# 294coder/Dif-PAN

Measured on AMD Instinct MI355X. Metric: fused megapixels/sec at T=1000, WV3 64x64x8 tiles, higher is better.
Workload: dtype f32-class (f16x2 split); 1 GPU; WV3 pansharpening, batch 64 of 64x64x8 tiles per GPU, T=1000 DDPM p_sample, fp32; tiles_per_gpu=64, tiles_total=64, T=1000, model_evaluations=1000, sampler=ddpm, parallelism=tile-shard x1, launches_per_denoising_step=132

## Files before the change

### dif-pan_amd/csrc/ddif_la.cpp

```cpp
#include "ddif_plan.h"
#include "kernels_lafuse.h"
#include "kernels_lafuse8.h"

namespace ddif {

namespace {
template <int TH, int TW, int NBQ, int NBA>
int la_launch1(const LaFuseArgs& a, int grid, hipStream_t s, bool prepare_only) {
    using G = LaFuseGeom<TH, TW, NBQ, NBA>;
    auto fn = linattn_fused_kernel<TH, TW, NBQ, NBA>;
    if (prepare_only) {
        DDIF_HIPCHK(hipFuncSetAttribute(reinterpret_cast<const void*>(fn), hipFuncAttributeMaxDynamicSharedMemorySize, (int)G::smem));
        return 0;
    }
    hipLaunchKernelGGL(fn, dim3(grid), dim3(2 * TH * TW), G::smem, s, a);
    return 0;
}
template <int TH, int TW>
int la_launch_t(const LaFuseArgs& a, int nbq, int nba, int grid, hipStream_t s, bool prep) {
    switch (nbq * 10 + nba) {
        case 21: return la_launch1<TH, TW, 2, 1>(a, grid, s, prep);
        case 31: return la_launch1<TH, TW, 3, 1>(a, grid, s, prep);
        case 41: return la_launch1<TH, TW, 4, 1>(a, grid, s, prep);
        case 22: return la_launch1<TH, TW, 2, 2>(a, grid, s, prep);
        case 32: return la_launch1<TH, TW, 3, 2>(a, grid, s, prep);
        case 42: return la_launch1<TH, TW, 4, 2>(a, grid, s, prep);
        case 62:
            if constexpr (TH == 16) return la_launch1<TH, TW, 6, 2>(a, grid, s, prep);
            [[fallthrough]];
        default: return fail(DDIF_ERR_INVALID, "linattn_fused: no instantiation for %d q blocks / %d output blocks", nbq, nba);
    }
}
}

bool lafuse_supported(int H, int fea, int dout) {
    static const bool la6 = env_flag("DDIF_LA6", true);
    if (H == 16 && fea == 192 && dout == 64 && la6) return true;
    return (H == 64 || H == 32 || H == 16) && fea % 32 == 0 && fea >= 64 && fea <= 128 && dout % 32 == 0 && dout >= 32 && dout <= 64;
}
int lafuse_strip(int H, int nw) { return 32 * nw / H; }
int lafuse_launch(const LaFuseArgs& a, int grid, hipStream_t s, bool prepare_only, int nw) {
    const int nbq = (a.c0 + a.c1) / 32, nba = a.dout / 32;
    if (nw == 4) {
        if (a.H == 64) return la_launch_t<64, 2>(a, nbq, nba, grid, s, prepare_only);
        if (a.H == 32) return la_launch_t<32, 4>(a, nbq, nba, grid, s, prepare_only);
        if (a.H == 16) return la_launch_t<16, 8>(a, nbq, nba, grid, s, prepare_only);
    } else {
        if (a.H == 64) return la_launch_t<64, 4>(a, nbq, nba, grid, s, prepare_only);
        if (a.H == 32) return la_launch_t<32, 8>(a, nbq, nba, grid, s, prepare_only);
        if (a.H == 16) return la_launch_t<16, 16>(a, nbq, nba, grid, s, prepare_only);
    }
    return fail(DDIF_ERR_INVALID, "linattn_fused: H = %d", a.H);
}

bool lafuse8_supported(int H, int W, int c0, int c1, int dout) {
    return H == 8 && W == 8 && c0 % 64 == 0 && c1 % 64 == 0 && (c0 + c1 == 256 || c0 + c1 == 192) && dout == 128;
}
int lafuse8_launch(const LaFuseArgs& a, int grid, hipStream_t s, bool prepare_only) {
    const int nbq = (a.c0 + a.c1) / 32;
    if (nbq == 8) {
        auto fn = linattn8_fused_kernel<8>;
        if (prepare_only) {
            DDIF_HIPCHK(hipFuncSetAttribute(reinterpret_cast<const void*>(fn), hipFuncAttributeMaxDynamicSharedMemorySize, (int)LaFuse8Geom<8>::smem));
            return 0;
        }
        hipLaunchKernelGGL(fn, dim3(grid), dim3(512), LaFuse8Geom<8>::smem, s, a);
        return 0;
    }
    if (nbq == 6) {
        auto fn = linattn8_fused_kernel<6>;
        if (prepare_only) {
            DDIF_HIPCHK(hipFuncSetAttribute(reinterpret_cast<const void*>(fn), hipFuncAttributeMaxDynamicSharedMemorySize, (int)LaFuse8Geom<6>::smem));
            return 0;
        }
        hipLaunchKernelGGL(fn, dim3(grid), dim3(512), LaFuse8Geom<6>::smem, s, a);
        return 0;
    }
    return fail(DDIF_ERR_INVALID, "linattn8_fused: %d feature channels", a.c0 + a.c1);
}

}
```

### dif-pan_amd/csrc/ddif_net.cpp

```cpp
#include "ddif_net.h"
#include <cstdint>
#include <tuple>
#include "kernels_refresh.h"

namespace ddif {

thread_local std::string g_err;

int fail(int code, const char* fmt, ...) {
    char buf[1024];
    va_list ap;
    va_start(ap, fmt);
    vsnprintf(buf, sizeof(buf), fmt, ap);
    va_end(ap);
    g_err = buf;
    return code;
}

static bool in_list(const int32_t* a, int n, int v) {
    for (int i = 0; i < n; ++i)
        if (a[i] == v) return true;
    return false;
}

// ... 96 lines not shown
    size_t n = 1;
    for (int i = 0; i < ndim; ++i) {
        if (shape[i] < 0) return fail(DDIF_ERR_INVALID, "ddif_net_load(%s): negative dim", key);
        t.shape.push_back(shape[i]);
        n *= (size_t)shape[i];
    }
    t.v.assign(data, data + n);
    host[key] = std::move(t);
    committed = false;
    return 0;
}

int64_t Net::num_params() const {
    int64_t n = 0;
    for (auto& kv : host)
        if (kv.first != "noise_level_mlp.0.freqs") n += (int64_t)kv.second.v.size();
    return n;
}

namespace {

struct Blob {
    std::vector<float> v;
    size_t add(const float* p, size_t n) {
        size_t off = (v.size() + 63) & ~(size_t)63;
        v.resize(off + n, 0.f);
        if (p) std::memcpy(v.data() + off, p, n * sizeof(float));
        return off;
    }
};

size_t pack_conv(Blob& b, const float* w, int cout, int cin, int ks, int ck, int* n_chunks_out) {
    const int n_chunks = (cin + ck - 1) / ck, nb = (cout + 31) / 32, nb_pad = (nb + 3) & ~3;
    const int taps = ks * ks, K8 = ck / 8;
    const size_t n = (size_t)nb_pad * n_chunks * taps * K8 * 256;
    const size_t off = b.add(nullptr, n);
    float* o = b.v.data() + off;
    for (int nbi = 0; nbi < nb; ++nbi)
        for (int ch = 0; ch < n_chunks; ++ch)
            for (int tap = 0; tap < taps; ++tap)
                for (int k8 = 0; k8 < K8; ++k8)
                    for (int h = 0; h < 2; ++h)
                        for (int j = 0; j < 32; ++j)
                            for (int i = 0; i < 4; ++i) {
                                const int ci = ch * ck + k8 * 8 + 4 * h + i, co = nbi * 32 + j;
                                float val = 0.f;
                                if (co < cout && ci < cin) val = w[((size_t)co * cin + ci) * taps + tap];
                                o[(((((size_t)nbi * n_chunks + ch) * taps + tap) * K8 + k8) * 2 + h) * 128 + j * 4 + i] = val;
                            }
    *n_chunks_out = n_chunks;
    return off;
}

inline unsigned bf16_bits_host(float x) {
    unsigned u;
    std::memcpy(&u, &x, 4);
    return (u + 0x7fffu + ((u >> 16) & 1u)) >> 16;
}
inline float bf16_val_host(unsigned b) {
    const unsigned u = b << 16;
    float f;
    std::memcpy(&f, &u, 4);
    return f;
}
size_t pack_conv_x3(Blob& b, const float* w, int cout, int cin, int ks, int ck) {
    const int taps = ks * ks, K16 = ck / 16;
    const int n_chunks = (cin + ck - 1) / ck, nb = (cout + 31) / 32, nb_pad = (nb + 3) & ~3;
    const size_t per = (size_t)taps * K16 * 3 * 256;
    const size_t off = b.add(nullptr, (size_t)nb_pad * n_chunks * per);
    uint16_t* o = reinterpret_cast<uint16_t*>(b.v.data() + off);
    for (int nbi = 0; nbi < nb; ++nbi)
        for (int ch = 0; ch < n_chunks; ++ch)
            for (int tap = 0; tap < taps; ++tap)
              for (int k16 = 0; k16 < K16; ++k16)
                for (int h = 0; h < 2; ++h)
                    for (int j = 0; j < 32; ++j)
                        for (int t = 0; t < 8; ++t) {
                            const int ci = ch * ck + 16 * k16 + 8 * h + t, co = nbi * 32 + j;
                            float val = 0.f;
                            if (co < cout && ci < cin) val = w[((size_t)co * cin + ci) * taps + tap];
                            unsigned q[3];
                            q[0] = bf16_bits_host(val);
                            const float r1 = val - bf16_val_host(q[0]);
                            q[1] = bf16_bits_host(r1);
                            q[2] = bf16_bits_host(r1 - bf16_val_host(q[1]));
                            for (int pl = 0; pl < 3; ++pl) {
                                const size_t fl = (((((size_t)nbi * n_chunks + ch) * taps + tap) * K16 + k16) * 3 + pl) * 256 + (size_t)(h * 32 + j) * 4;
                                o[fl * 2 + t] = (uint16_t)q[pl];
                            }
                        }
    return off;
}

inline uint16_t f16_bits_host(float x) {
    const _Float16 hv = (_Float16)x;
    uint16_t b;
    std::memcpy(&b, &hv, 2);
    return b;
}
inline float f16_val_host(uint16_t b) {
    _Float16 hv;
    std::memcpy(&hv, &b, 2);
    return (float)hv;
}
size_t pack_conv_f16(Blob& b, const float* w, int cout, int cin, int ks, int ck) {
    const int taps = ks * ks, K16 = ck / 16;
    for (size_t i = 0; i < (size_t)cout * cin * taps; ++i)
        if (!(std::fabs(w[i]) <= DDIF_F16_WMAX)) return (size_t)-1;
    const int n_chunks = (cin + ck - 1) / ck, nb = (cout + 31) / 32, nb_pad = (nb + 3) & ~3;
    const size_t per = (size_t)taps * K16 * 2 * 256;
    const size_t off = b.add(nullptr, (size_t)nb_pad * n_chunks * per);
    uint16_t* o = reinterpret_cast<uint16_t*>(b.v.data() + off);
    for (int nbi = 0; nbi < nb; ++nbi)
        for (int ch = 0; ch < n_chunks; ++ch)
            for (int tap = 0; tap < taps; ++tap)
                for (int k16 = 0; k16 < K16; ++k16)
                    for (int h = 0; h < 2; ++h)
                        for (int j = 0; j < 32; ++j)
                            for (int t = 0; t < 8; ++t) {
                                const int ci = ch * ck + 16 * k16 + 8 * h + t, co = nbi * 32 + j;
                                float val = 0.f;
                                if (co < cout && ci < cin) val = w[((size_t)co * cin + ci) * taps + tap] * DDIF_F16_WSCALE;
                                uint16_t q[2];
                                q[0] = f16_bits_host(val);
                                q[1] = f16_bits_host(val - f16_val_host(q[0]));
                                for (int pl = 0; pl < 2; ++pl) {
                                    const size_t fl = (((((size_t)nbi * n_chunks + ch) * taps + tap) * K16 + k16) * 2 + pl) * 256 + (size_t)(h * 32 + j) * 4;
                                    o[fl * 2 + t] = q[pl];
                                }
                            }
    return off;
}

size_t pack_conv_b1(Blob& b, size_t x3_off, int cout, int cin, int ks, int ck) {
    const size_t steps = (size_t)((((cout + 31) / 32 + 3) & ~3)) * ((cin + ck - 1) / ck) * (ks * ks) * (ck / 16);
    const size_t off = b.add(nullptr, steps * 256);
    for (size_t st = 0; st < steps; ++st) std::memcpy(b.v.data() + off + st * 256, b.v.data() + x3_off + st * 3 * 256, 256 * sizeof(float));
    return off;
}

}

int Net::commit(hipStream_t stream) {
    Blob b;
    struct PendConv { std::string name; size_t w_off; long bias_off; int cin, cout, ks, ck, n_chunks; long x3_off = -1; long f16_off = -1; long b1_off = -1; };
    std::vector<PendConv> pend;
    std::map<std::string, size_t> vec_off;
    std::string missing;
    recipes.clear();
    auto rec_pack = [&](int kind, const std::string& s0, const std::string& s1, size_t off, int cout, int cin0, int cin1, int ks, int ck, int n_chunks) {
        Recipe r;
        r.kind = kind;
        r.src0 = s0;
        r.src1 = s1;
        r.dst_off = off;
        r.cout = cout;
        r.cin0 = cin0;
        r.cin1 = cin1;
        r.ks = ks;
        r.ck = ck;
        r.n_chunks = n_chunks;
        const size_t nb_pad = (size_t)(((cout + 31) / 32 + 3) & ~3);
        r.n_out = kind == RF_PACK_F32 ? nb_pad * n_chunks * ks * ks * (ck / 8) * 256 : nb_pad * n_chunks * ks * ks * (ck / 16) * 3 * 256;
        recipes.push_back(r);
    };
    auto rec_copy = [&](int kind, const std::string& s0, const std::string& s1, size_t off, size_t n, int C = 0) {
        Recipe r;
        r.kind = kind;
        r.src0 = s0;
        r.src1 = s1;
        r.dst_off = off;
        r.n_out = n;
        r.cout = C;
        recipes.push_back(r);
    };

    auto need = [&](const std::string& key) -> const HostTensor* {
        const HostTensor* t = get(key);
        if (!t && missing.empty()) missing = key;
        return t;
    };
    auto add_conv = [&](const std::string& name, bool has_bias) {
        const HostTensor* w = need(name + ".weight");
        const HostTensor* bs = has_bias ? need(name + ".bias") : nullptr;
        if (!w || (has_bias && !bs)) return;
        if (w->shape.size() != 4) { if (missing.empty()) missing = name + ".weight (expected 4-d)"; return; }
        PendConv p;
        p.name = name;
        p.cout = (int)w->shape[0];
        p.cin = (int)w->shape[1];
        p.ks = (int)w->shape[2];
        p.ck = (p.ks == 3 || p.cin <= 16) ? 16 : 32;
        p.w_off = pack_conv(b, w->v.data(), p.cout, p.cin, p.ks, p.ck, &p.n_chunks);
        rec_pack(RF_PACK_F32, name + ".weight", "", p.w_off, p.cout, p.cin, 0, p.ks, p.ck, p.n_chunks);
        if (p.ck % 16 == 0 && (p.ks == 3 || p.ck == 32)) {
            p.x3_off = (long)pack_conv_x3(b, w->v.data(), p.cout, p.cin, p.ks, p.ck);
            rec_pack(RF_PACK_X3, name + ".weight", "", (size_t)p.x3_off, p.cout, p.cin, 0, p.ks, p.ck, p.n_chunks);
            p.f16_off = (long)pack_conv_f16(b, w->v.data(), p.cout, p.cin, p.ks, p.ck);
            p.b1_off = (long)pack_conv_b1(b, (size_t)p.x3_off, p.cout, p.cin, p.ks, p.ck);
        }
        p.bias_off = bs ? (long)b.add(bs->v.data(), bs->v.size()) : -1;
        if (bs) rec_copy(RF_COPY, name + ".bias", "", (size_t)p.bias_off, bs->v.size());
        pend.push_back(p);
    };
    auto add_vec = [&](const std::string& key) {
        const HostTensor* t = need(key);
        if (t) {
            vec_off[key] = b.add(t->v.data(), t->v.size());
            rec_copy(RF_COPY, key, "", vec_off[key], t->v.size());
        }
    };
    auto add_dw = [&](const std::string& key) {
        const HostTensor* t = need(key);
        if (!t) return;
        const int C = (int)t->shape[0];
        std::vector<float> r((size_t)9 * C);
        for (int c = 0; c < C; ++c)
            for (int k = 0; k < 9; ++k) r[(size_t)k * C + c] = t->v[(size_t)c * 9 + k];
        vec_off[key] = b.add(r.data(), r.size());
        rec_copy(RF_DW, key, "", vec_off[key], r.size(), C);
    };
    auto add_resblock = [&](const std::string& p) {
        add_vec(p + ".block1.block.0.weight");
        add_vec(p + ".block1.block.0.bias");
        add_conv(p + ".block1.block.3", true);
        add_vec(p + ".block2.block.0.weight");
        add_vec(p + ".block2.block.0.bias");
        add_conv(p + ".block2.block.3", true);
    };
    auto add_attn = [&](const std::string& p) {
        add_vec(p + ".norm.weight");
        add_vec(p + ".norm.bias");
        add_conv(p + ".qkv", false);
        add_conv(p + ".out", true);
    };

    std::vector<float> wall_h, ball_h;
    std::vector<std::tuple<std::string, size_t, size_t, size_t, size_t>> slot_keys;
    slot_off.clear();
    nslots = 0;
    auto add_slot = [&](const std::string& rb) {
        const HostTensor* w = need(rb + ".noise_func.noise_func.0.weight");
        const HostTensor* bs = need(rb + ".noise_func.noise_func.0.bias");
        if (!w || !bs) return;
        slot_off[rb] = nslots;
        slot_keys.emplace_back(rb, wall_h.size(), (size_t)nslots, w->v.size(), bs->v.size());
        wall_h.insert(wall_h.end(), w->v.begin(), w->v.end());
        ball_h.insert(ball_h.end(), bs->v.begin(), bs->v.end());
        nslots += (int)bs->v.size();
    };

    for (auto& L : downs) {
        if (L.kind == L_STEM) add_conv(L.p, true);
        else if (L.kind == L_DOWN) add_conv(L.p + ".conv", true);
        else {
            add_slot(L.p + ".res_block");
            add_resblock(L.p + ".res_block");
            if (L.attn) add_attn(L.p + ".attn");
            add_conv(L.p + ".cond_inj.body.0", false);
            add_vec(L.p + ".cond_inj.body.1.weight");
            add_vec(L.p + ".cond_inj.body.1.bias");
            add_conv(L.p + ".cond_inj.body.3", true);
            add_conv(L.p + ".cond_inj.x_conv", true);
            if (const HostTensor* wx = get(L.p + ".cond_inj.x_conv.weight")) {
                if (wx->shape.size() == 4 && wx->shape[1] == 32 && wx->shape[0] % 32 == 0 && wx->shape[2] == 1) {
                    const int co = (int)wx->shape[0];
                    std::vector<float> r((size_t)co * 32);
                    for (int nb = 0; nb < co / 32; ++nb)
                        for (int ln = 0; ln < 64; ++ln)
                            for (int sx = 0; sx < 16; ++sx)
                                r[((size_t)nb * 64 + ln) * 16 + sx] = wx->v[(size_t)(32 * nb + (ln & 31)) * 32 + 8 * (sx >> 2) + 4 * (ln >> 5) + (sx & 3)];
                    vec_off[L.p + ".cond_inj.x_conv.xf"] = b.add(r.data(), r.size());
                }
            }
        }
    }
    for (auto& L : mid) {
        add_slot(L.p + ".res_block");
        add_resblock(L.p + ".res_block");
        if (L.attn) add_attn(L.p + ".attn");
    }
    for (auto& L : ups) {
        if (L.kind == L_UP) { add_conv(L.p + ".conv", true); continue; }
        add_slot(L.p + ".res_block");
        add_resblock(L.p + ".res_block");
        if (L.attn) add_attn(L.p + ".attn");
        const std::string ci = L.p + ".cond_inj";
        add_vec(ci + ".prenorm_x.weight");
        add_vec(ci + ".prenorm_x.bias");
        add_dw(ci + ".q.0.weight");
        add_conv(ci + ".q.1", true);
        add_dw(ci + ".kv.0.weight");
        add_conv(ci + ".kv.1", true);
        const HostTensor *wo = need(ci + ".attn_out.weight"), *bo = need(ci + ".attn_out.bias");
        const HostTensor* wr = get(ci + ".attn_res.weight");
        const HostTensor* br = get(ci + ".attn_res.bias");
        if (wo) {
            vec_off[ci + ".attn_out.weight"] = b.add(wo->v.data(), wo->v.size());
            rec_copy(RF_COPY, ci + ".attn_out.weight", "", vec_off[ci + ".attn_out.weight"], wo->v.size());
        }
        if (wr) {
            vec_off[ci + ".attn_res.weight"] = b.add(wr->v.data(), wr->v.size());
            rec_copy(RF_COPY, ci + ".attn_res.weight", "", vec_off[ci + ".attn_res.weight"], wr->v.size());
        }
        if (wo && bo) {
            const int co = (int)wo->shape[0], fea = (int)wo->shape[1];
            PendConv p;
            p.name = ci + ".attn_mix";
            p.cout = co;
            p.ks = 1;
            std::vector<float> bsum(bo->v);
            if (wr && br) {
                std::vector<float> cat((size_t)co * 2 * fea);
                for (int o = 0; o < co; ++o) {
                    std::memcpy(&cat[(size_t)o * 2 * fea], &wo->v[(size_t)o * fea], fea * sizeof(float));
                    std::memcpy(&cat[(size_t)o * 2 * fea + fea], &wr->v[(size_t)o * fea], fea * sizeof(float));
                    bsum[o] = bo->v[o] + br->v[o];
                }
                p.cin = 2 * fea;
                p.ck = 32;
                p.w_off = pack_conv(b, cat.data(), co, p.cin, 1, p.ck, &p.n_chunks);
                rec_pack(RF_PACK_F32, ci + ".attn_out.weight", ci + ".attn_res.weight", p.w_off, co, fea, fea, 1, p.ck, p.n_chunks);
                p.x3_off = (long)pack_conv_x3(b, cat.data(), co, p.cin, 1, p.ck);
                rec_pack(RF_PACK_X3, ci + ".attn_out.weight", ci + ".attn_res.weight", (size_t)p.x3_off, co, fea, fea, 1, p.ck, p.n_chunks);
                p.b1_off = (long)pack_conv_b1(b, (size_t)p.x3_off, co, p.cin, 1, p.ck);
            } else {
                p.cin = fea;
                p.ck = fea <= 16 ? 16 : 32;
                p.w_off = pack_conv(b, wo->v.data(), co, fea, 1, p.ck, &p.n_chunks);
                rec_pack(RF_PACK_F32, ci + ".attn_out.weight", "", p.w_off, co, fea, 0, 1, p.ck, p.n_chunks);
                if (p.ck == 32) {
                    p.x3_off = (long)pack_conv_x3(b, wo->v.data(), co, fea, 1, p.ck);
                    rec_pack(RF_PACK_X3, ci + ".attn_out.weight", "", (size_t)p.x3_off, co, fea, 0, 1, p.ck, p.n_chunks);
                    p.b1_off = (long)pack_conv_b1(b, (size_t)p.x3_off, co, fea, 1, p.ck);
                }
            }
            p.bias_off = (long)b.add(bsum.data(), bsum.size());
            if (wr && br) rec_copy(RF_SUM, ci + ".attn_out.bias", ci + ".attn_res.bias", (size_t)p.bias_off, bsum.size());
            else rec_copy(RF_COPY, ci + ".attn_out.bias", "", (size_t)p.bias_off, bsum.size());
            pend.push_back(p);
        }
        add_conv(ci + ".ffn.0", false);
        add_conv(ci + ".ffn.2", false);
        add_conv(ci + ".ffn.3", true);
        {
            const HostTensor *w2 = get(ci + ".ffn.2.weight"), *w3 = get(ci + ".ffn.3.weight"), *b3 = get(ci + ".ffn.3.bias");
            if (w2 && w3 && b3 && w2->shape.size() == 4 && w3->shape.size() == 4 && w3->shape[1] == w2->shape[0] && w3->shape[2] == 1) {
                const int co = (int)w3->shape[0], mid = (int)w2->shape[0], cin = (int)w2->shape[1];
                std::vector<float> wm((size_t)co * cin * 9);
                std::vector<double> row((size_t)cin * 9);
                for (int o = 0; o < co; ++o) {
                    std::fill(row.begin(), row.end(), 0.0);
                    for (int k = 0; k < mid; ++k) {
                        const double a = (double)w3->v[(size_t)o * mid + k];
                        const float* src = &w2->v[(size_t)k * cin * 9];
                        for (int e = 0; e < cin * 9; ++e) row[e] += a * (double)src[e];
                    }
                    for (int e = 0; e < cin * 9; ++e) wm[(size_t)o * cin * 9 + e] = (float)row[e];
                }
                PendConv p;
                p.name = ci + ".ffn.23";
                p.cout = co;
                p.cin = cin;
                p.ks = 3;
                p.ck = 16;
                p.w_off = pack_conv(b, wm.data(), co, cin, 3, p.ck, &p.n_chunks);
                p.x3_off = (long)pack_conv_x3(b, wm.data(), co, cin, 3, p.ck);
                p.f16_off = (long)pack_conv_f16(b, wm.data(), co, cin, 3, p.ck);
                p.b1_off = (long)pack_conv_b1(b, (size_t)p.x3_off, co, cin, 3, p.ck);
                p.bias_off = (long)b.add(b3->v.data(), b3->v.size());
                pend.push_back(p);
            }
        }
    }
    add_vec("final_conv.block.0.weight");
    add_vec("final_conv.block.0.bias");
    add_conv("final_conv.block.3", true);

    const HostTensor *hw1 = need("noise_level_mlp.1.weight"), *hb1 = need("noise_level_mlp.1.bias");
    const HostTensor *hw3 = need("noise_level_mlp.3.weight"), *hb3 = need("noise_level_mlp.3.bias");
    if (!missing.empty()) return fail(DDIF_ERR_MISSING, "ddif_net_commit: weight '%s' was never loaded", missing.c_str());

    const int half = cfg.inner_channel / 2;
    std::vector<float> fr(half);
    if (const HostTensor* f = get("noise_level_mlp.0.freqs")) {
        if ((int)f->v.size() != half) return fail(DDIF_ERR_INVALID, "noise_level_mlp.0.freqs must have %d entries", half);
        fr = f->v;
    } else {
        const float k = -(float)std::log(1e4);
        for (int j = 0; j < half; ++j) fr[j] = std::exp(k * ((float)j / (float)half));
    }
    const size_t o_fr = b.add(fr.data(), fr.size());
    const size_t o_w1 = b.add(hw1->v.data(), hw1->v.size()), o_b1 = b.add(hb1->v.data(), hb1->v.size());
    const size_t o_w3 = b.add(hw3->v.data(), hw3->v.size()), o_b3 = b.add(hb3->v.data(), hb3->v.size());
    const size_t o_wall = b.add(wall_h.data(), wall_h.size()), o_ball = b.add(ball_h.data(), ball_h.size());
    rec_copy(RF_COPY, "noise_level_mlp.1.weight", "", o_w1, hw1->v.size());
    rec_copy(RF_COPY, "noise_level_mlp.1.bias", "", o_b1, hb1->v.size());
    rec_copy(RF_COPY, "noise_level_mlp.3.weight", "", o_w3, hw3->v.size());
    rec_copy(RF_COPY, "noise_level_mlp.3.bias", "", o_b3, hb3->v.size());
    for (auto& sk : slot_keys) {
        rec_copy(RF_COPY, std::get<0>(sk) + ".noise_func.noise_func.0.weight", "", o_wall + std::get<1>(sk), std::get<3>(sk));
        rec_copy(RF_COPY, std::get<0>(sk) + ".noise_func.noise_func.0.bias", "", o_ball + std::get<2>(sk), std::get<4>(sk));
    }
    merged_stale = false;
    last_ptrs.clear();
    refresh_keys.clear();
    dconv.clear();
    dgrad_filled = false;
    if (blob || dgrad_blob) {
        for (hipEvent_t e : reader_events) DDIF_HIPCHK(hipEventSynchronize(e));
        DDIF_HIPCHK(hipStreamSynchronize(stream));
    }
    if (dgrad_blob) {
        DDIF_HIPCHK(hipFree(dgrad_blob));
        dgrad_blob = nullptr;
    }

    if (blob) {
        DDIF_HIPCHK(hipFree(blob));
        blob = nullptr;
    }
    blob_floats = b.v.size() + 64;
    DDIF_HIPCHK(hipMalloc((void**)&blob, blob_floats * sizeof(float)));
    DDIF_HIPCHK(hipMemcpy(blob, b.v.data(), b.v.size() * sizeof(float), hipMemcpyHostToDevice));
    (void)stream;

    conv.clear();
    vec.clear();
    for (auto& p : pend) {
        PackedConv pc;
        pc.w = blob + p.w_off;
        pc.w_x3 = p.x3_off >= 0 ? blob + p.x3_off : nullptr;
        pc.w_f16 = p.f16_off >= 0 ? blob + p.f16_off : nullptr;
        pc.w_b1 = p.b1_off >= 0 ? blob + p.b1_off : nullptr;
        pc.bias = p.bias_off >= 0 ? blob + p.bias_off : nullptr;
        pc.cin = p.cin;
        pc.cout = p.cout;
        pc.ks = p.ks;
        pc.ck = p.ck;
        pc.n_chunks = p.n_chunks;
        conv[p.name] = pc;
    }
    vec_absmax.clear();
    for (auto& kv : vec_off) {
        vec[kv.first] = blob + kv.second;
        float m = 0.f;
        if (const HostTensor* t = get(kv.first))
            for (float x : t->v) m = std::fabs(x) > m || std::isnan(x) ? (std::isnan(x) ? INFINITY : std::fabs(x)) : m;
        vec_absmax[blob + kv.second] = m;
    }
    freqs = blob + o_fr;
    w1 = blob + o_w1;
    b1 = blob + o_b1;
    w3 = blob + o_w3;
    b3 = blob + o_b3;
    wall = blob + o_wall;
    ball = blob + o_ball;
    committed = true;
    ++generation;
    return 0;
}

int Net::refresh_device(int n, const char* const* keys, const float* const* ptrs, hipStream_t stream) {
    if (!committed) return fail(DDIF_ERR_STATE, "ddif_net_refresh: ddif_net_commit has not been called");
    if (n < 1 || !keys || !ptrs) return fail(DDIF_ERR_INVALID, "ddif_net_refresh: bad arguments");
#ifndef DDIF_EMU
    for (hipEvent_t e : reader_events) (void)hipStreamWaitEvent(stream, e, 0);
#endif
    bool same = (int)refresh_keys.size() == n && d_recs != nullptr;
    for (int i = 0; i < n && same; ++i) {
        if (!keys[i] || !ptrs[i]) return fail(DDIF_ERR_INVALID, "ddif_net_refresh: NULL key / pointer at %d", i);
        same = refresh_in_ptrs[i] == ptrs[i] && refresh_keys[i] == keys[i];
    }
    if (same) {
        hipLaunchKernelGGL(refresh_blob_kernel, dim3((unsigned)refresh_blocks), dim3(256), 0, stream, (const RefreshRec*)d_recs, n_recs);
        DDIF_HIPCHK(hipGetLastError());
        merged_stale = true;
        if (dgrad_blob) dgrad_filled = true;
        return 0;
    }
    std::map<std::string, const float*> by_key;
    for (int i = 0; i < n; ++i) {
        if (!keys[i] || !ptrs[i]) return fail(DDIF_ERR_INVALID, "ddif_net_refresh: NULL key / pointer at %d", i);
        by_key[keys[i]] = ptrs[i];
    }
    refresh_keys.clear();
    std::vector<const float*> flat;
    flat.reserve(recipes.size() * 2);
    for (auto& r : recipes) {
        auto i0 = by_key.find(r.src0);
        if (i0 == by_key.end()) return fail(DDIF_ERR_MISSING, "ddif_net_refresh: parameter '%s' was not given", r.src0.c_str());
        const float* p1 = nullptr;
        if (!r.src1.empty()) {
            auto i1 = by_key.find(r.src1);
            if (i1 == by_key.end()) return fail(DDIF_ERR_MISSING, "ddif_net_refresh: parameter '%s' was not given", r.src1.c_str());
            p1 = i1->second;
        }
        flat.push_back(i0->second);
        flat.push_back(p1);
    }
    if (flat != last_ptrs || !d_recs) {
        std::vector<RefreshRec> recs(recipes.size());
        long long blk = 0;
        for (size_t k = 0; k < recipes.size(); ++k) {
            const Recipe& r = recipes[k];
            RefreshRec& d = recs[k];
            d.kind = r.kind;
            d.src0 = flat[2 * k];
            d.src1 = flat[2 * k + 1];
            d.dst = (r.dblob ? dgrad_blob : blob) + r.dst_off;
            d.tr = r.tr;
            d.fc0 = r.fc0;
            d.fc1 = r.fc1;
            d.cout = r.cout;
            d.cin0 = r.cin0;
            d.cin1 = r.cin1;
            d.ks = r.ks;
            d.ck = r.ck;
            d.n_chunks = r.n_chunks;
            d.n_out = (long long)r.n_out;
            d.blk0 = blk;
            blk += (long long)((r.n_out + 255) / 256);
        }
        if (d_recs) {
            DDIF_HIPCHK(hipStreamSynchronize(stream));
            DDIF_HIPCHK(hipFree(d_recs));
            d_recs = nullptr;
        }
        DDIF_HIPCHK(hipMalloc(&d_recs, recs.size() * sizeof(RefreshRec)));
        DDIF_HIPCHK(hipMemcpy(d_recs, recs.data(), recs.size() * sizeof(RefreshRec), hipMemcpyHostToDevice));
        n_recs = (int)recs.size();
        refresh_blocks = blk;
        last_ptrs = flat;
    }
    refresh_keys.assign(keys, keys + n);
    refresh_in_ptrs.assign(ptrs, ptrs + n);
    hipLaunchKernelGGL(refresh_blob_kernel, dim3((unsigned)refresh_blocks), dim3(256), 0, stream, (const RefreshRec*)d_recs, n_recs);
    DDIF_HIPCHK(hipGetLastError());
    merged_stale = true;
    if (dgrad_blob) dgrad_filled = true;
    return 0;
}

int Net::build_dgrad_packs() {
    if (!committed) return fail(DDIF_ERR_STATE, "build_dgrad_packs: ddif_net_commit has not been called");
    if (dgrad_blob) return 0;
    size_t off = 0;
    std::vector<Recipe> extra;
    auto add = [&](const std::string& name, const std::string& s0, const std::string& s1, int cout_f, int fc0, int fc1, int ks) {
        PackedConv pc;
        pc.cin = cout_f;
        pc.cout = (fc0 + fc1 + 3) & ~3;
        pc.ks = ks;
        pc.ck = (ks == 3 || pc.cin <= 16) ? 16 : 32;
        pc.n_chunks = (pc.cin + pc.ck - 1) / pc.ck;
        const size_t nb_pad = (size_t)(((pc.cout + 31) / 32 + 3) & ~3);
        const bool x3 = pc.ck % 16 == 0 && (ks == 3 || pc.ck == 32);
        Recipe r;
        r.kind = RF_PACK_F32;
        r.src0 = s0;
        r.src1 = s1;
        r.cout = pc.cout;
        r.cin0 = cout_f;
        r.ks = ks;
        r.ck = pc.ck;
        r.n_chunks = pc.n_chunks;
        r.tr = 1;
        r.fc0 = fc0;
        r.fc1 = fc1;
        r.dblob = true;
        r.dst_off = off;
        r.n_out = nb_pad * pc.n_chunks * ks * ks * (pc.ck / 8) * 256;
        const size_t w_off = off;
        off += (r.n_out + 63) & ~(size_t)63;
        extra.push_back(r);
        size_t x3_off = 0;
        if (x3) {
            Recipe q = r;
            q.kind = RF_PACK_X3;
            q.dst_off = off;
            q.n_out = nb_pad * pc.n_chunks * ks * ks * (pc.ck / 16) * 3 * 256;
            x3_off = off;
            off += (q.n_out + 63) & ~(size_t)63;
            extra.push_back(q);
        }
        pc.w = reinterpret_cast<const float*>(w_off + 1);
        pc.w_x3 = x3 ? reinterpret_cast<const float*>(x3_off + 1) : nullptr;
        pc.bias = nullptr;
        dconv[name] = pc;
    };
    for (auto& kv : conv) {
        const std::string& name = kv.first;
        const PackedConv& f = kv.second;
        const size_t n = name.size();
        auto ends = [&](const char* suf) { const size_t m = strlen(suf); return n >= m && name.compare(n - m, m, suf) == 0; };
        if (ends(".ffn.23") || ends(".body.0") || name == "downs.0") continue;
        if (ends(".attn_mix")) {
            const std::string ci = name.substr(0, n - strlen(".attn_mix"));
            const bool has_res = get(ci + ".attn_res.weight") != nullptr;
            const int fea = has_res ? f.cin / 2 : f.cin;
            add(name, ci + ".attn_out.weight", has_res ? ci + ".attn_res.weight" : "", f.cout, fea, has_res ? fea : 0, 1);
            continue;
        }
        add(name, name + ".weight", "", f.cout, f.cin, 0, f.ks);
    }
    dgrad_floats = off + 64;
// ... 16 lines not shown
```

### dif-pan_amd/csrc/ddif_plan.cpp

```cpp
#include "ddif_plan.h"
#include <algorithm>
#include "kernels_conv.h"
#include "kernels_misc.h"
#include "attn_args.h"
#include "quantile_args.h"
#include "kernels_lafuse.h"

namespace ddif {

ConvVariant get_conv_variant(int ks, int stride, int ups, int ck, int pro, int cfg, int vec, int epi, int math) {
    if (cfg == 20 || cfg == 21)
        return (stride == 1 && !ups && vec == 1) ? get_lr_variant(ks, cfg == 20 ? 2 : 4, pro, epi, (math == MATH_F16X2 && pro == PRO_COLSM) ? MATH_BF16X3 : math) : ConvVariant();
    if (ks == 1) return get_conv_variant_k1(stride, ups, ck, pro, cfg, vec, epi);
    if (ks == 3) return epi ? get_conv_variant_k3e(stride, ups, ck, pro, cfg, vec, epi) : get_conv_variant_k3(stride, ups, ck, pro, cfg, vec);
    return ConvVariant();
}

static int num_cus();
static int x3_enabled() { static const int v = env_int("DDIF_X3", 1); return v; }
static int f16_enabled() { static const int v = env_int("DDIF_F16", 1); return v; }
int g_math_mode = [] { const char* e = getenv("DDIF_MATH"); return (e && std::strcmp(e, "bf16") == 0) ? 1 : 0; }();
int g_f16_raw = env_flag("DDIF_F16_RAW", true);
static int lr_rows_enabled() { static const int v = env_int("DDIF_LR_ROWS", 1); return v; }
static int lafuse_enabled() { static const int v = env_int("DDIF_LAFUSE", 1); return v; }
// ... 917 lines not shown
        s.stats = true;
        s.name = "up";
        const Tensor uin = cur;
        DDIF_TRY(p.add_conv(step, s, &cur));
        --lev;
        if (train) tmod(Plan::TrainMod::UP, L.p + ".conv", uin, cur);
        return 0;
    }
    struct Dec {
        std::string ci;
        Tensor skip;
        int skip_from = -1;
        int fea = 0, d = 0, Hl = 0, Wl = 0, cd = 0;
        size_t pre_dec0 = 0;
        float* ctx = nullptr;
        Tensor kdw, kv;
        const float *pn_g = nullptr, *pn_b = nullptr, *q0w = nullptr;
    };
    int decoder_context(Dec& D) {
        const int BB = B, fea = D.fea, d = D.d, Hl = D.Hl, Wl = D.Wl, cd = D.cd;
        D.pre_dec0 = pre.size();
        DDIF_TRY(p.alloc_tensor(&D.kdw, cd, Hl, Wl));
        {
            DwArgs a{};
            a.in0 = p.cdec[lev].p;
            a.c0 = cd;
            a.B = B;
            a.H = Hl;
            a.W = Wl;
            a.w = V(D.ci + ".kv.0.weight");
            if (!a.w) return fail(DDIF_ERR_MISSING, "%s.kv.0.weight missing", D.ci.c_str());
            a.out_dw = D.kdw.p;
            a.tiles_x = (Wl + 15) / 16;
            a.tiles_y = (Hl + 7) / 8;
            Op op;
            op.name = "kv.dw3x3";
            op.flop = 2.0 * 9 * B * Hl * Wl * cd;
            op.bytes = 8.0 * B * Hl * Wl * cd;
            op.run = [a](hipStream_t s, const StepCtx&) { launch_dw3x3(s, a); };
            pre.push_back(std::move(op));
        }
        ConvSpec s;
        DDIF_TRY(need_conv(D.ci + ".kv.1", &s.pc));
        s.in0 = D.kdw;
        s.name = "kv.1x1";
        DDIF_TRY(p.add_conv(pre, s, &D.kv));
        if (train) return 0;
        float *kmx = nullptr, *ksm = nullptr, *ctx = nullptr;
        DDIF_TRY(p.dalloc(&kmx, (size_t)B * Hl * fea));
        DDIF_TRY(p.dalloc(&ksm, (size_t)B * Hl * fea));
        DDIF_TRY(p.dalloc(&ctx, (size_t)B * 8 * d * d));
        D.ctx = ctx;
        const Tensor kv = D.kv;
        {
            Op op;
            op.name = "k.softmax_stats";
            op.bytes = 8.0 * B * Hl * Wl * fea;
            op.run = [kv, kmx, ksm, fea, BB, Hl, Wl](hipStream_t s, const StepCtx&) {
                hipLaunchKernelGGL(softmax_stats_kernel, ew_grid((size_t)BB * Hl * fea), dim3(256), 0, s, (const float*)kv.p, 2 * fea, 0, fea, BB, Hl, Wl, 1, kmx, ksm);
            };
            pre.push_back(std::move(op));
        }
        {
            Op op;
            op.name = "linattn_ctx";
            op.flop = 2.0 * B * 8 * d * d * (double)Hl * Wl;
            op.bytes = 4.0 * B * Hl * Wl * 2.0 * fea;
            op.run = [kv, kmx, ksm, ctx, fea, d, BB, Hl, Wl](hipStream_t s, const StepCtx&) {
                hipLaunchKernelGGL(linattn_ctx_kernel, dim3(8, BB), dim3(256), 2 * 32 * d * sizeof(float), s, (const float*)kv.p, (const float*)kmx, (const float*)ksm, BB, Hl, Wl, fea, d, ctx);
            };
            pre.push_back(std::move(op));
        }
        return 0;
    }
    DwArgs gn_dw_args(const Dec& D, Tensor dwq, Tensor xn) const {
        DwArgs a{};
        a.in0 = cur.p;
        a.c0 = cur.C;
        a.in1 = D.skip.p;
        a.c1 = D.skip.C;
        a.B = B;
        a.H = D.Hl;
        a.W = D.Wl;
        a.st0 = cur.st;
        a.np0 = cur.np;
        a.st1 = D.skip.st;
        a.np1 = D.skip.np;
        a.gamma = D.pn_g;
        a.beta = D.pn_b;
        a.w = D.q0w;
        a.out_dw = dwq.p;
        a.out_xn = xn.p;
        a.use_gn = 1;
        return a;
    }
    void pack_mix_weights(const Dec& D, const float* wo, const float* wr, float* wmix, int co_n, int ck, int nch, int nb_pad, size_t per, bool x3) {
        Op op;
        op.name = "pack_mix_weights";
        const float scale = 1.0f / std::sqrt((float)D.d);
        const int BB = B, fea = D.fea, d = D.d;
        const float* ctx = D.ctx;
        op.flop = 2.0 * B * co_n * (double)fea * d;
        op.run = [wo, wr, ctx, wmix, BB, co_n, fea, d, scale, ck, nch, nb_pad, per, x3](hipStream_t s, const StepCtx&) {
            if (x3) hipLaunchKernelGGL(pack_mix_weights_x3_kernel, ew_grid(per * BB), dim3(256), 0, s, wo, wr, (const float*)ctx, BB, co_n, fea, d, scale, ck, nch, nb_pad, wmix);
            else hipLaunchKernelGGL(pack_mix_weights_kernel, ew_grid(per * BB), dim3(256), 0, s, wo, wr, (const float*)ctx, BB, co_n, fea, d, scale, ck, nch, nb_pad, wmix);
        };
        pre.push_back(std::move(op));
    }
    int ffn_train(const Dec& D, Tensor a, Tensor* f0, Tensor* f1, Tensor* f2, Tensor* f3c) {
        const int Hl = D.Hl, Wl = D.Wl;
        ConvSpec s;
        DDIF_TRY(need_conv(D.ci + ".ffn.0", &s.pc));
        s.in0 = a;
        s.use_bias = false;
        s.name = "ffn.0 (train)";
        DDIF_TRY(p.add_conv(step, s, f0));
        DDIF_TRY(p.alloc_tensor(f1, f0->C, f0->H, f0->W, true));
        Op op;
        op.name = "silu";
        op.cls = cls_small(Hl * Wl, 5);
        op.bytes = 8.0 * B * Hl * Wl * f0->C;
        Tensor ff0 = *f0, ff1 = *f1;
        const size_t n = (size_t)B * Hl * Wl * f0->C;
        op.run = [ff0, ff1, n](hipStream_t st, const StepCtx&) { tk::silu_fwd(st, ff0.p, n, ff1.p); };
        step.push_back(std::move(op));
        ConvSpec s2;
        DDIF_TRY(need_conv(D.ci + ".ffn.2", &s2.pc));
        s2.in0 = *f1;
        s2.use_bias = false;
        s2.name = "ffn.2 (train)";
        DDIF_TRY(p.add_conv(step, s2, f2));
        ConvSpec s3;
        DDIF_TRY(need_conv(D.ci + ".ffn.3", &s3.pc));
        s3.in0 = *f2;
        s3.name = "ffn.3 (train)";
        return p.add_conv(step, s3, f3c);
    }
    int droppath_add(Tensor f3c, Tensor a, Tensor* out, float** scale_out) {
        Tensor f3;
        float* scale = nullptr;
        DDIF_TRY(p.alloc_tensor(&f3, f3c.C, f3c.H, f3c.W, true));
        DDIF_TRY(p.dalloc(&scale, (size_t)B));
        p.path_sites.push_back(scale);
        const int HW = f3c.H * f3c.W, Cc = f3c.C, BB = B;
        int chunks = (HW * Cc / 4 + 256 * 8 - 1) / (256 * 8);
        if (chunks < 1) chunks = 1;
        f3.np = chunks;
        DDIF_TRY(p.dalloc(&f3.st, (size_t)B * chunks * 2));
        Op op;
        op.name = "droppath_add";
        op.cls = cls_small(HW, 5);
        op.bytes = 12.0 * B * HW * Cc;
        op.run = [f3c, scale, a, f3, HW, Cc, BB, chunks](hipStream_t s, const StepCtx&) {
            hipLaunchKernelGGL(droppath_add_kernel, dim3(chunks, BB), dim3(256), 64, s, (const float*)f3c.p, (const float*)scale, (const float*)a.p, HW, Cc, f3.p, f3.st);
        };
        step.push_back(std::move(op));
        *out = f3;
        *scale_out = scale;
        return 0;
    }
    int decoder_block_train(const Dec& D, Tensor* out) {
        const std::string& ci = D.ci;
        const int BB = B, fea = D.fea, d = D.d, Hl = D.Hl, Wl = D.Wl;
        const PackedConv* pq1t = PC(ci + ".q.1");
        const PackedConv* pmixt = PC(ci + ".attn_mix");
        if (!pq1t || !pmixt) return fail(DDIF_ERR_MISSING, "%s: q.1 / attn_out missing", ci.c_str());
        if (!cur.st || !D.skip.st) return fail(DDIF_ERR_STATE, "%s: prenorm without producer statistics", ci.c_str());
        if (!D.pn_g || !D.pn_b || !D.q0w) return fail(DDIF_ERR_MISSING, "%s: prenorm/q.0 weights missing", ci.c_str());
        Tensor xn, dwq, q, o, a, f0, f1, f2, f3c, f3, kdw_pad;
        float *la_ctx = nullptr, *la_part = nullptr;
        DDIF_TRY(p.alloc_tensor(&xn, fea, Hl, Wl, true));
        DDIF_TRY(p.alloc_tensor(&dwq, fea, Hl, Wl, true));
        {
            DwArgs da = gn_dw_args(D, dwq, xn);
            da.tiles_x = (Wl + 15) / 16;
            da.tiles_y = (Hl + 7) / 8;
            Op op;
            op.name = "q.gn_dw3x3 (train)";
            op.cls = cls_small(Hl * Wl, 5);
            op.flop = 2.0 * 9 * B * Hl * Wl * fea;
            op.bytes = 12.0 * B * Hl * Wl * fea;
            op.run = [da](hipStream_t s, const StepCtx&) { launch_dw3x3(s, da); };
            step.push_back(std::move(op));
        }
        {
            ConvSpec s;
            s.pc = pq1t;
            s.in0 = dwq;
            s.name = "q.1x1 (train)";
            DDIF_TRY(p.add_conv(step, s, &q));
        }
        DDIF_TRY(p.alloc_tensor(&o, fea, Hl, Wl, true));
        {
            Op op;
            op.name = "linattn_fwd";
            op.cls = cls_small(Hl * Wl, 5);
            op.flop = 4.0 * B * 8 * d * d * (double)Hl * Wl;
            op.bytes = 16.0 * B * Hl * Wl * fea;
            Tensor qq = q, kk = D.kv, oo = o;
            if ((Hl > Wl ? Hl : Wl) * fea > 8192 || d > 32 || d % 4)
                return fail(DDIF_ERR_INVALID, "%s: train-mode linear attention holds one image line x %d channels in LDS: lines of more than %d pixels are not supported",
                            ci.c_str(), fea, 8192 / fea);
            DDIF_TRY(p.dalloc(&la_ctx, (size_t)B * fea * d));
            DDIF_TRY(p.dalloc(&la_part, tk::linattn_part_floats(B, Hl, Wl, fea, d)));
            float *cx = la_ctx, *pt = la_part;
            {
                Op pc;
                pc.name = "linattn_ctx (train)";
                pc.bytes = 8.0 * B * Hl * Wl * fea;
                pc.run = [kk, BB, d, Hl, Wl, cx, pt](hipStream_t s, const StepCtx&) { tk::linattn_ctx(s, kk.p, BB, 8, d, Hl, Wl, cx, pt); };
                pre.push_back(std::move(pc));
                for (size_t i = D.pre_dec0; i < pre.size(); ++i) pre[i].side = true;
            }
            op.run = [qq, oo, BB, d, Hl, Wl, fea, cx](hipStream_t s, const StepCtx&) { tk::linattn_apply(s, qq.p, cx, BB, 8, d, Hl, Wl, oo.p, fea); };
            step.push_back(std::move(op));
        }
        const bool has_res = pmixt->cin == 2 * fea;
        {
            ConvSpec s;
            s.pc = pmixt;
            s.in0 = o;
            if (has_res) s.in1 = xn;
            else s.res = xn.p;
            s.name = "attn_out+res (train)";
            DDIF_TRY(p.add_conv(step, s, &a));
        }
        DDIF_TRY(ffn_train(D, a, &f0, &f1, &f2, &f3c));
        float* scale = nullptr;
        DDIF_TRY(droppath_add(f3c, a, &f3, &scale));
        DDIF_TRY(p.alloc_tensor(&kdw_pad, (D.cd + 3) & ~3, Hl, Wl));
        Plan::TrainMod& m = tmod(Plan::TrainMod::DEC, ci, cur, f3);
        m.t[0] = D.skip;
        m.t[1] = xn;
        m.t[2] = dwq;
        m.t[3] = q;
        m.t[4] = D.kv;
        m.t[5] = D.kdw;
        m.t[6] = kdw_pad;
        m.t[7] = o;
        m.t[8] = a;
        m.t[9] = f0;
        m.t[10] = f1;
        m.t[11] = f2;
        m.scale = scale;
        m.ctx = la_ctx;
        m.la_part = la_part;
        m.has_res = has_res;
        m.skip_from = D.skip_from;
        m.lev = lev;
        *out = f3;
        return 0;
    }
    int linattn_fused(const Dec& D, const PackedConv* pq1, Tensor* amix, bool* fused) {
        const std::string& ci = D.ci;
        const int fea = D.fea, Hl = D.Hl, Wl = D.Wl;
        const Tensor& skip = D.skip;
        *fused = false;
        const PackedConv* pm = PC(ci + ".attn_mix");
        const float* wr = V(ci + ".attn_res.weight");
        const bool la8 = la8_enabled() && lafuse8_supported(Hl, Wl, cur.C, skip.C, pm ? pm->cout : 0);
        bool ok = lafuse_enabled() && f16_enabled() && x3_enabled() && lr_enabled() && pm && wr && pq1->w_f16 && pq1->bias && pm->bias && (Hl * Wl >= 256 || la8) &&
                  pq1->cout == fea && pq1->ck == 32 && pm->ck == 32 && pm->cin == 2 * fea && cur.C % 16 == 0 && skip.C % 16 == 0 && (la8 || lafuse_supported(Hl, fea, pm->cout));
        if (ok) {
            auto ig = net.vec_absmax.find(D.pn_g), ib = net.vec_absmax.find(D.pn_b), iw = net.vec_absmax.find(D.q0w);
            ok = ig != net.vec_absmax.end() && ib != net.vec_absmax.end() && iw != net.vec_absmax.end() &&
                 (std::sqrt((double)fea * Hl * Wl) * ig->second + ib->second) * 9.0 * iw->second < DDIF_F16_AMAX;
        }
        if (!ok) return 0;
        const float* wo = V(ci + ".attn_out.weight");
        if (!wo) return fail(DDIF_ERR_MISSING, "%s.attn_out.weight missing", ci.c_str());
        const int nb_pad = (((pm->cout + 31) / 32) + 3) & ~3;
        const size_t per = (size_t)nb_pad * pm->n_chunks * 2 * 3 * 256;
        float* wmix = nullptr;
        DDIF_TRY(p.dalloc(&wmix, per * B));
        pack_mix_weights(D, wo, wr, wmix, pm->cout, 32, pm->n_chunks, nb_pad, per, true);
        p.use(cur.p);
        p.use(skip.p);
        DDIF_TRY(p.alloc_tensor(amix, pm->cout, Hl, Wl, true));
        LaFuseArgs a{};
        a.xcd = (xcd_mask() & 4) ? 1 : 0;
        a.in0 = cur.p;
        a.c0 = cur.C;
        a.in1 = skip.p;
        a.c1 = skip.C;
        a.B = B;
        a.H = Hl;
        a.W = Wl;
        a.st0 = cur.st;
        a.np0 = cur.np;
        a.st1 = skip.st;
        a.np1 = skip.np;
        a.gamma = D.pn_g;
        a.beta = D.pn_b;
        a.dw_w = D.q0w;
        a.wq = pq1->w_f16;
        a.nchq = pq1->n_chunks;
        a.bq = pq1->bias;
        a.wmix = wmix;
        a.wmix_bstride = (long long)per;
        a.nch_mix = pm->n_chunks;
        a.bias = pm->bias;
        a.out = amix->p;
        a.dout = pm->cout;
        int la_nw = 8;
        if (!la8) {
            static const int nw_env = env_int("DDIF_LA_NW", 0);
            const long wg8 = (long)B * ((Wl + lafuse_strip(Hl, 8) - 1) / lafuse_strip(Hl, 8));
            la_nw = nw_env == 4 || nw_env == 8 ? nw_env : (wg8 < num_cus() ? 4 : 8);
        }
        if (!p.dry) DDIF_TRY(la8 ? lafuse8_launch(a, 1, nullptr, true) : lafuse_launch(a, 1, nullptr, true, la_nw));
        const int nstrips = la8 ? 2 : (Wl + lafuse_strip(Hl, la_nw) - 1) / lafuse_strip(Hl, la_nw);
        long cap = num_cus();
        if (g_debug_grid_cap > 0 && g_debug_grid_cap < cap) cap = g_debug_grid_cap;
        Op op;
        op.name = la8 ? "linattn8_fused" : "linattn_fused";
        {
            char lb[160];
            snprintf(lb, sizeof lb, "linattn_fused GN+dw3x3+q.1+softmax_H+attn_out+res %d+%d->%d @%dx%d", cur.C, skip.C, pm->cout, Hl, Wl);
            op.label = lb;
        }
        op.flop = 2.0 * B * Hl * Wl * ((double)fea * fea + 9.0 * fea + 2.0 * fea * pm->cout);
        op.bytes = 4.0 * B * Hl * Wl * ((double)fea + pm->cout);
        op.cls = cls_small(Hl * Wl, 1);
        op.mfma_w = (3.0 * fea * fea + 6.0 * 2.0 * fea * pm->cout) / ((double)fea * fea + 9.0 * fea + 2.0 * fea * pm->cout);
        op.run = [a, nstrips, cap, la8, la_nw](hipStream_t st, const StepCtx&) {
            const long nw = (long)a.B * nstrips;
            if (la8) (void)lafuse8_launch(a, (int)(nw < cap ? nw : cap), st, false);
            else (void)lafuse_launch(a, (int)(nw < cap ? nw : cap), st, false, la_nw);
        };
        step.push_back(std::move(op));
        *fused = true;
        return 0;
    }
    int q_low_resolution(const Dec& D, const PackedConv* pq1, Tensor xn, Tensor* q, float** qmx, float** qsm) {
        const int BB = B, fea = D.fea, Hl = D.Hl, Wl = D.Wl;
        Tensor dwq;
        DDIF_TRY(p.alloc_tensor(&dwq, fea, Hl, Wl, true));
        p.use(cur.p);
        p.use(D.skip.p);
        p.use(xn.p);
        DwArgs a = gn_dw_args(D, dwq, xn);
        Op op;
        op.name = "q.gn_dw3x3";
        op.cls = 2;
        {
            char lb[160];
            snprintf(lb, sizeof lb, "q.gn_dw3x3 %d+%d @%dx%d", cur.C, D.skip.C, Hl, Wl);
            op.label = lb;
        }
        op.flop = 2.0 * 9 * B * Hl * Wl * fea;
        op.bytes = 4.0 * B * Hl * Wl * 3.0 * fea;
        const size_t sm = (size_t)(Hl + 2) * (Wl + 2) * 36 * sizeof(float);
        if (sm > 64 * 1024) DDIF_HIPCHK(hipFuncSetAttribute(reinterpret_cast<const void*>(gn_dw3x3_small_kernel), hipFuncAttributeMaxDynamicSharedMemorySize, (int)sm));
        a.xcd = (xcd_mask() & 8) ? 1 : 0;
        const dim3 gdw = a.xcd ? dim3(BB, (fea + 31) / 32) : dim3((fea + 31) / 32, BB);
        op.run = [a, gdw, sm](hipStream_t s, const StepCtx&) { hipLaunchKernelGGL(gn_dw3x3_small_kernel, gdw, dim3(256), sm, s, a); };
        step.push_back(std::move(op));
        ConvSpec s;
        s.pc = pq1;
        s.in0 = dwq;
        s.name = "q.1x1";
        if (Hl <= 16) {
            DDIF_TRY(p.dalloc(qmx, (size_t)B * Wl * fea));
            DDIF_TRY(p.dalloc(qsm, (size_t)B * Wl * fea));
            s.cso_mx = *qmx;
            s.cso_sm = *qsm;
            s.name = "q.1x1 (+softmax_H stats)";
        }
        return p.add_conv(step, s, q);
    }
    int linattn_three_launch(const Dec& D, const PackedConv* pq1, Tensor* amix) {
        const std::string& ci = D.ci;
        const int BB = B, fea = D.fea, Hl = D.Hl, Wl = D.Wl;
        const Tensor& skip = D.skip;
        Tensor xn, q;
        DDIF_TRY(p.alloc_tensor(&xn, fea, Hl, Wl, true));
        if (pq1->ck != 32 || cur.C % 4 != 0 || skip.C % 4 != 0 || fea > 256)
            return fail(DDIF_ERR_INVALID, "%s: the fused q = 1x1(dw3x3(GN(cat))) kernel needs 4 | channels and <= 256 of them (got %d+%d)", ci.c_str(), cur.C, skip.C);
        float *qmx = nullptr, *qsm = nullptr;
        if (pick_cfg(CfgQuery{1, 32, PRO_NONE, 1, 1, 0, Hl, Wl, pq1->cout, B, fea, fea}) >= 20) {
            DDIF_TRY(q_low_resolution(D, pq1, xn, &q, &qmx, &qsm));
        } else {
            ConvSpec s;
            s.pc = pq1;
            s.in0 = cur;
            s.in1 = skip;
            s.pro = PRO_GN_DW;
            s.gamma = D.pn_g;
            s.beta = D.pn_b;
            s.dw_w = D.q0w;
            s.out_xn = xn.p;
            s.name = "q = 1x1(dw3x3(GN(cat)))";
            DDIF_TRY(p.add_conv(step, s, &q));
        }
        if (!qmx) {
            DDIF_TRY(p.dalloc(&qmx, (size_t)B * Wl * fea));
            DDIF_TRY(p.dalloc(&qsm, (size_t)B * Wl * fea));
            p.use(q.p);
            Op op;
            op.name = "q.softmax_stats";
            op.cls = 4;
            op.bytes = 8.0 * B * Hl * Wl * fea;
            op.run = [q, qmx, qsm, fea, BB, Hl, Wl](hipStream_t s, const StepCtx&) {
                hipLaunchKernelGGL(softmax_stats_kernel, ew_grid((size_t)BB * Wl * fea), dim3(256), 0, s, (const float*)q.p, fea, 0, fea, BB, Hl, Wl, 0, qmx, qsm);
            };
            step.push_back(std::move(op));
        }
        const PackedConv* pmix = PC(ci + ".attn_mix");
        if (!pmix) return fail(DDIF_ERR_MISSING, "%s.attn_out missing", ci.c_str());
        if (fea % 32 != 0 || pmix->ck != 32) return fail(DDIF_ERR_INVALID, "%s: linear attention over %d channels needs 32 | channels", ci.c_str(), fea);
        const int nb_pad = (((pmix->cout + 31) / 32) + 3) & ~3;
        const bool mix_x3 = pick_cfg(CfgQuery{1, pmix->ck, PRO_COLSM, 1, 1, 0, Hl, Wl, pmix->cout, B, pmix->cin, pmix->cin == 2 * fea ? fea : pmix->cin}) >= 12;
        const size_t per = mix_x3 ? (size_t)nb_pad * pmix->n_chunks * (pmix->ck / 16) * 3 * 256 : (size_t)nb_pad * pmix->n_chunks * (pmix->ck / 8) * 256;
        float* wmix = nullptr;
        DDIF_TRY(p.dalloc(&wmix, per * B));
        const float* wo = V(ci + ".attn_out.weight");
        const float* wr = V(ci + ".attn_res.weight");
        if (!wo) return fail(DDIF_ERR_MISSING, "%s.attn_out.weight missing", ci.c_str());
        pack_mix_weights(D, wo, wr, wmix, pmix->cout, pmix->ck, pmix->n_chunks, nb_pad, per, mix_x3);
        ConvSpec s;
        s.pc = pmix;
        s.in0 = q;
        if (pmix->cin == 2 * fea) s.in1 = xn;
        else s.res = xn.p;
        s.pro = PRO_COLSM;
        s.cs_mx = qmx;
        s.cs_sm = qsm;
        s.w_override = wmix;
        s.w_bstride = (long long)per;
        s.name = "softmax_H(q).ctx.attn_out+res";
        return p.add_conv(step, s, amix);
    }
    int ffn(const Dec& D, Tensor amix, Tensor* f3) {
        Tensor f1, f2;
        ConvSpec s;
        DDIF_TRY(need_conv(D.ci + ".ffn.0", &s.pc));
        s.in0 = amix;
        s.use_bias = false;
        s.silu = true;
        s.name = "ffn.0";
        DDIF_TRY(p.add_conv(step, s, &f1));
        ConvSpec s2;
        DDIF_TRY(need_conv(D.ci + ".ffn.2", &s2.pc));
        s2.in0 = f1;
        s2.use_bias = false;
        s2.name = "ffn.2";
        ConvSpec s3;
        DDIF_TRY(need_conv(D.ci + ".ffn.3", &s3.pc));
        if (const PackedConv* pm = PC(D.ci + ".ffn.23")) {
            ConvSpec sf = s2;
            sf.pc = pm;
            sf.use_bias = true;
            sf.res = amix.p;
            sf.stats = true;
            sf.name = "ffn.3(ffn.2) merged + res";
            return p.add_conv(step, sf, f3);
        }
        DDIF_TRY(p.add_conv(step, s2, &f2));
        s3.in0 = f2;
        s3.res = amix.p;
        s3.stats = true;
        s3.name = "ffn.3";
        return p.add_conv(step, s3, f3);
    }
    int decoder_block(const Layer& L) {
        Dec D;
        D.ci = L.p + ".cond_inj";
        D.skip = feats.back();
        feats.pop_back();
        if (train) {
            D.skip_from = feat_mod.back();
            feat_mod.pop_back();
        }
        if (D.skip.C != L.cskip || cur.C != L.cx || D.skip.H != cur.H || D.skip.W != cur.W)
            return fail(DDIF_ERR_INVALID, "%s: skip/feature shape mismatch", L.p.c_str());
        D.fea = L.cin;
        D.d = D.fea / 8;
        D.Hl = cur.H;
        D.Wl = cur.W;
        D.cd = Cl + 3 * Pn;
        DDIF_TRY(decoder_context(D));
        const std::string& ci = D.ci;
        D.pn_g = V(ci + ".prenorm_x.weight");
        D.pn_b = V(ci + ".prenorm_x.bias");
        D.q0w = V(ci + ".q.0.weight");
        Tensor f3;
        if (train) {
            DDIF_TRY(decoder_block_train(D, &f3));
        } else {
            const PackedConv* pq1 = PC(ci + ".q.1");
            if (!pq1) return fail(DDIF_ERR_MISSING, "%s.q.1 missing", ci.c_str());
            if (!cur.st || !D.skip.st) return fail(DDIF_ERR_STATE, "%s: prenorm without producer statistics", ci.c_str());
            if (!D.pn_g || !D.pn_b || !D.q0w) return fail(DDIF_ERR_MISSING, "%s: prenorm/q.0 weights missing", ci.c_str());
            p.tap(ci + ".cur", cur);
            p.tap(ci + ".skip", D.skip);
            p.tap(ci + ".cond", p.cdec[lev], true);
            Tensor amix;
            bool fused_attn = false;
            DDIF_TRY(linattn_fused(D, pq1, &amix, &fused_attn));
            if (!fused_attn) DDIF_TRY(linattn_three_launch(D, pq1, &amix));
            p.tap(ci + ".a", amix);
            DDIF_TRY(ffn(D, amix, &f3));
            p.tap(ci + ".out", f3);
        }
        DDIF_TRY(resblock(L.p + ".res_block", f3, &cur));
        return attention_if(L);
    }
    int final_conv() {
        ConvSpec s;
        DDIF_TRY(need_conv("final_conv.block.3", &s.pc));
        s.in0 = cur;
        s.pro = PRO_GN_SILU;
        s.gamma = V("final_conv.block.0.weight");
        s.beta = V("final_conv.block.0.bias");
        s.name = "final";
        s.samp = true;
        DDIF_TRY(p.add_conv(step, s, &p.net_out));
        if (train) tmod(Plan::TrainMod::FINAL, "final_conv", cur, p.net_out);
        return 0;
    }
};
}

int Plan::build_impl() {
    const ddif_net_cfg& c = net->cfg;
    if (!net->committed) return fail(DDIF_ERR_STATE, "ddif_plan_create: ddif_net_commit has not been called");
    C = c.out_channel;
    P = c.pan_channel;
    CC = 2 * c.lms_channel + 4 * P;
    const int nlev = c.n_channel_mults;
    const int div = 1 << (nlev - 1);
    if (B < 1 || H < div || W < div || H % div || W % div)
        return fail(DDIF_ERR_INVALID, "ddif_plan_create: H=%d W=%d must be positive multiples of %d", H, W, div);
    LH.assign(1, H);
    LW.assign(1, W);
    for (int l = 1; l < nlev; ++l) {
        LH.push_back((LH.back() - 1) / 2 + 1);
        LW.push_back((LW.back() - 1) / 2 + 1);
    }
    PlanBuilder b(*this);
    DDIF_TRY(b.boundary_buffers());
    DDIF_TRY(b.cond_program());
    for (size_t li = 0; li < net->downs.size(); ++li) {
        const Layer& L = net->downs[li];
        DDIF_TRY(L.kind == L_STEM ? b.stem(li) : (L.kind == L_DOWN ? b.down(li) : b.encoder_block(li)));
        tap(L.p, b.cur);
        b.feats.push_back(b.cur);
        if (train_mode) {
            tmods.back().pushes_feat = true;
            b.feat_mod.push_back((int)tmods.size() - 1);
        }
    }
    for (const Layer& L : net->mid) {
        DDIF_TRY(b.mid_block(L));
        tap(L.p, b.cur);
    }
    if (train_mode) b.join_side_stream();
    for (const Layer& L : net->ups) {
        DDIF_TRY(L.kind == L_UP ? b.up(L) : b.decoder_block(L));
        tap(L.p, b.cur);
    }
    DDIF_TRY(b.final_conv());
    DDIF_TRY(ensure_tb(B));
    return 0;
}
#undef DDIF_TRY

void Plan::drop_graphs() {
#ifndef DDIF_EMU
    for (auto& g : graph_exec) {
        if (g) (void)hipGraphExecDestroy((hipGraphExec_t)g);
        g = nullptr;
    }
#endif
}

int Plan::ensure_tb(int rows) {
    if (rows <= tb_rows) return 0;
    drop_graphs();
    if (int e = dalloc(&tb, (size_t)rows * net->nslots)) return e;
    if (int e = dalloc(&tvals, (size_t)rows)) return e;
    tb_rows = rows;
    return 0;
}

int Plan::time_rows(const float* t_host, int rows, hipStream_t s) { return time_rows_aux(t_host, rows, nullptr, s); }

static int check_sampler_net(const Net* n);

int Plan::time_rows_aux(const float* t_host, int rows, float* aux, hipStream_t s) {
    if (int e = ensure_tb(rows)) return e;
    DDIF_HIPCHK(hipMemcpyAsync(tvals, t_host, (size_t)rows * sizeof(float), hipMemcpyDefault, s));
    const int inner = net->cfg.inner_channel;
    hipLaunchKernelGGL(time_embed_kernel, dim3(rows), dim3(128), (size_t)6 * inner * sizeof(float), s, (const float*)tvals,
                       net->freqs, net->w1, net->b1, net->w3, net->b3, net->wall, net->ball, inner, net->nslots, tb, aux);
    return 0;
}

namespace tk {
void dw3x3_plain(hipStream_t s, const float* in, int C, int B, int H, int W, const float* w9c, float* out, bool flip) {
    DwArgs a{};
    a.flip = flip ? 1 : 0;
    a.in0 = in;
    a.c0 = C;
    a.B = B;
    a.H = H;
    a.W = W;
    a.w = w9c;
    a.out_dw = out;
    a.tiles_x = (W + 15) / 16;
    a.tiles_y = (H + 7) / 8;
    launch_dw3x3(s, a);
}
}

int Plan::train_step(const float* x0, const float* noise, const float* a_h, const float* s_h, const float* t_h, const float* sc, float* loss_dev, float* pred,
                     hipStream_t s, const ddif_objective_rows* rows, float* recon_out) {
    if (!train_mode || bwd.empty()) return fail(DDIF_ERR_STATE, "ddif_plan_train_step: not a train-mode plan");
    if (!cond_set) return fail(DDIF_ERR_STATE, "ddif_plan_train_step before ddif_plan_set_cond");
    if (!x0 || !noise || !a_h || !s_h || !t_h) return fail(DDIF_ERR_INVALID, "ddif_plan_train_step: NULL argument");
    for (auto& kv : grad_slots)
        if (!kv.second) return fail(DDIF_ERR_STATE, "ddif_plan_train_step: gradient tensors are not bound (ddif_plan_train_bind); first missing: %s", kv.first.c_str());
    if (int e = check_sampler_net(net)) return e;
    const int HW = H * W;
    const size_t n = (size_t)B * HW * C;
    DDIF_HIPCHK(hipMemcpyAsync(small, a_h, (size_t)B * sizeof(float), hipMemcpyDefault, s));
    DDIF_HIPCHK(hipMemcpyAsync(small + B, s_h, (size_t)B * sizeof(float), hipMemcpyDefault, s));
    hipLaunchKernelGGL(nchw_to_nhwc_kernel, ew_grid(n), dim3(256), 0, s, x0, B, C, HW, 0, C, img[0]);
    hipLaunchKernelGGL(nchw_to_nhwc_kernel, ew_grid(n), dim3(256), 0, s, noise, B, C, HW, 0, C, img[1]);
    const bool p2 = rows && rows->p2_weight;
    if (pred_mode != DDIF_PRED_X_START || p2 || recon_out)
// ... 582 lines not shown
```

### dif-pan_amd/csrc/ddif_plan.h

```cpp
#pragma once
#include <cstdlib>
#include <string>
#include <memory>
#include "ddif_net.h"

namespace ddif {

inline int env_int(const char* name, int dflt) { const char* e = getenv(name); return e ? atoi(e) : dflt; }
inline bool env_flag(const char* name, bool dflt) { return env_int(name, dflt ? 1 : 0) != 0; }
bool train_x3();

struct ConvArgs;

struct Tensor {
    float* p = nullptr;
    int C = 0, H = 0, W = 0;
    double* st = nullptr;
    int np = 0;
};

struct StepCtx {
    const float* x = nullptr;
    const float* sc = nullptr;
    const float* tb = nullptr;
    int tb_stride = 0;
    const int* step_ptr = nullptr;
    int tb_rowstride = 0;
    float* samp_out = nullptr;
    const void* samp_run = nullptr;
    int* step_next = nullptr;
    int samp_kind = 0;
    bool samp_pred = false;
};

struct Op {
    std::function<void(hipStream_t, const StepCtx&)> run;
    double flop = 0, bytes = 0;
    double mfma_w = 16;
    bool timed = false;
    bool side = false;
    int cls = 5;
    const char* name = "";
    std::string label;
};

typedef void (*ConvKernelFn)(ConvArgs);
struct ConvVariant {
    ConvKernelFn fn = nullptr;
    size_t smem = 0;
    int th = 0, tw = 0, nt = 0, nthr = 256;
    bool x3 = false;
    bool f16 = false;
    bool b1 = false;
    int wg_cap = 2;
    bool lr = false;
    bool wr = false;
    const char* name = "";
};
enum { MATH_BF16X3 = 0, MATH_F16X2 = 1, MATH_BF16X1 = 2 };
ConvVariant get_conv_variant(int ks, int stride, int ups, int ck, int pro, int cfg, int vec, int epi, int math = MATH_BF16X3);
ConvVariant get_lr_variant(int ks, int mb, int pro, int epi, int math = MATH_BF16X3, bool rows = false);
ConvVariant get_conv_variant_k1(int stride, int ups, int ck, int pro, int cfg, int vec, int epi);
ConvVariant get_conv_variant_k3(int stride, int ups, int ck, int pro, int cfg, int vec);
ConvVariant get_conv_variant_k3e(int stride, int ups, int ck, int pro, int cfg, int vec, int epi);
ConvVariant get_xf_variant(int stride, int pro, int cfg, int vec, int epi, int nbx);
extern int g_math_mode;
extern int g_f16_raw;
struct LaFuseArgs;
bool lafuse_supported(int H, int fea, int dout);
int lafuse_strip(int H, int nw = 8);
int lafuse_launch(const LaFuseArgs& a, int grid, hipStream_t s, bool prepare_only, int nw = 8);
bool lafuse8_supported(int H, int W, int c0, int c1, int dout);
int lafuse8_launch(const LaFuseArgs& a, int grid, hipStream_t s, bool prepare_only);
namespace tk {
void film_apply(hipStream_t s, const float* xc, const float* film, int B, int HW, int C, float* out, double* st_out, int chunks);
int film_chunks(int HW, int C);
size_t linattn_part_floats(int B, int H, int W, int C, int d);
void linattn_fwd(hipStream_t s, const float* q, const float* kv, int B, int heads, int d, int H, int W, float* out, int ld_o, float* ctx, float* part);
void linattn_ctx(hipStream_t s, const float* kv, int B, int heads, int d, int H, int W, float* ctx, float* part);
void linattn_apply(hipStream_t s, const float* q, const float* ctx, int B, int heads, int d, int H, int W, float* out, int ld_o);
void linattn_bwd(hipStream_t s, const float* q, const float* kv, const float* dout, int ld_g, const float* ctx, int B, int heads, int d, int H, int W, float* dq, float* dkv,
                 float* dctx, float* part);
void linattn_bwd_q(hipStream_t s, const float* q, const float* dout, int ld_g, const float* ctx, int B, int heads, int d, int H, int W, float* dq, float* dctx, float* part);
void linattn_bwd_k(hipStream_t s, const float* kv, const float* dctx, int B, int heads, int d, int H, int W, float* dkv);
int linattn_prepare();
void silu_fwd(hipStream_t s, const float* x, size_t n, float* y);
void silu_bwd(hipStream_t s, const float* x, const float* da, size_t n, float* dx);
struct WgradGeom { int n_co = 0, n_ci = 0, nsplit = 0, rb = 0, nbchunk = 0, pf = 0, centre = 0; size_t smem = 0, partial_floats = 0;
                   int x3 = 0, xw = 0, ys = 0, xs = 0; };
WgradGeom wgrad_geom(int B, int Cin, int Cout, int H, int W, bool centre = false);
int wgrad_prepare();
void wgrad(hipStream_t s, const float* x, const float* dy, int B, int H, int W, int Cin, int Cout, const WgradGeom& g, bool centre, float* partial, float* dw,
           float* bpart = nullptr, float* db = nullptr);
void bias_grad(hipStream_t s, const float* dy, size_t npix, int Cout, int nbchunk, float* bpart, float* db);
void gn_stats(hipStream_t s, const float* x, int B, size_t per_sample, int nchunk, double* spart);
void gn_act(hipStream_t s, const float* x, const double* st, int np, const float* gamma, const float* beta, const float* mask, int B, int HW, int C, int silu, float* out);
void gn_bwd(hipStream_t s, const float* x, const float* da, const float* mask, const double* st, int np, const float* gamma, const float* beta, int B, int HW, int C,
            int nchunk, int silu, double* cpart, float* S, float* dgamma, float* dbeta, const float* res, float* dx, double* gpart = nullptr);
void gn_bwd_reduce_all(hipStream_t s, const GnRedRec* recs_dev, int nrec, int nblocks, int B);
void gn_bwd_cat(hipStream_t s, const float* x0, int c0, const float* x1, int c1, const double* st0, int np0, const double* st1, int np1, const float* da, const float* gamma,
                const float* beta, int B, int HW, int nchunk, double* cpart, float* S, float* dgamma, float* dbeta, float* dx0, float* dx1, double* gpart = nullptr);
void linear_bwd(hipStream_t s, const float* x, const float* w, const float* dy, int B, int nin, int nout, float* dx, float* dw, float* db);
void l1_fwd(hipStream_t s, const float* pred, const float* target, size_t n, float* out);
void l1_bwd(hipStream_t s, const float* pred, const float* target, size_t n, float upstream, float* dpred);
size_t ssimloss_workgroups(int B, int C, int H, int W);
int ssimloss_check(const char* who, int B, int C, int H, int W);
void ssimloss_tail(hipStream_t s, const float* img1, const float* img2, int B, int C, int H, int W, bool nhwc, float w_l1, float w_ssim, float upstream, const float* p2w,
                   float* maps, double* part, float* d_loss, float* d_img2);
void dw3x3_plain(hipStream_t s, const float* in, int C, int B, int H, int W, const float* w9c, float* out, bool flip = false);
}
struct AttnBlockArgs;
int attn_block_prepare();
void attn_block_launch(const AttnBlockArgs& a, int grid, hipStream_t s);
int attn_block_split();
bool attn_block_has_f16();

struct XfReq {
    const PackedConv* pc = nullptr;
    const float* w = nullptr;
    const float* film = nullptr;
    Tensor out;
    bool done = false;
};

struct ConvSpec {
    const PackedConv* pc = nullptr;
    Tensor in0, in1;
    bool dyn_input = false;
    int stride = 1, ups = 0, pro = PRO_NONE;
    const float* gamma = nullptr;
    const float* beta = nullptr;
    bool use_bias = true;
    int tb_off = -1;
    const float* res = nullptr;
    const float* film = nullptr;
    const float* w_override = nullptr;
    long long w_bstride = 0;
    const float* cs_mx = nullptr;
    const float* cs_sm = nullptr;
    const float* dw_w = nullptr;
    float* out_xn = nullptr;
    float* cso_mx = nullptr;
    float* cso_sm = nullptr;
    bool silu = false;
    bool stats = false;
    bool exact = false;
    bool samp = false;
    XfReq* xf = nullptr;
    const char* name = "conv";
};

struct Plan {
    Net* net = nullptr;
    unsigned long long generation = 0;
    int B = 0, H = 0, W = 0, C = 0, P = 0, CC = 0;
    std::vector<void*> allocs;
    std::vector<Op> pre, step;
    bool cond_set = false;
    bool train_mode = false;
    struct DropSite { float* mask; int C, H, W; };
    std::vector<DropSite> drop_sites;
    std::vector<float*> path_sites;
    float* mask_recs = nullptr;
    int n_mask_recs = 0;
    unsigned long long mask_blocks = 0;
    size_t bytes_allocated = 0;

    float* cond_nchw = nullptr;
    Tensor lms;
    std::vector<Tensor> cenc, cdec;
    std::vector<int> LH, LW;
    Tensor x_in, sc_in, net_out;
    float* zeros = nullptr;
    float* img[2] = {nullptr, nullptr};
    float* mbuf[3] = {nullptr, nullptr, nullptr};
    float* io_nchw = nullptr;
    float* tvals = nullptr;
    float* tb = nullptr;
    int tb_rows = 0;
    float* small = nullptr;
    int* d_step = nullptr;
    bool final_fused_pred = false;
    int pred_mode = DDIF_PRED_X_START, loss_type = DDIF_LOSS_L1;
    int set_objective(int pred, int loss);
    float w_l1 = 1.0f, w_ssim = 0.1f;
    float* ssim_maps = nullptr;
    double* ssim_part = nullptr;
    int thr_mode = DDIF_THRESHOLD_OFF;
    float thr_ratio = 0.f, thr_max = 1.f;
    float* d_thr = nullptr;
    bool graph_dyn = false;
    int set_threshold(int mode, float ratio, float max_val);
    bool final_fused = false;
    int math_mode = 0;
    int f16_raw = 1;
    int* d_range = nullptr;
    int n_range_convs = 0;
    int range_status(hipStream_t s, int* overflow);
    void* d_run = nullptr;
    float* d_tabs = nullptr;
    int tabs_cap = 0;
    hipStream_t cap_stream = nullptr;
    void* graph_exec[2] = {nullptr, nullptr};
    bool use_graph = true;

    int prof_every = 0, prof_max = 0;
    bool prof_all = false;
    std::vector<hipEvent_t> ev0, ev1;
    std::vector<double> ev_flop, ev_bytes, ev_mflop;
    std::vector<int> ev_cls;
    int ev_used = 0;
    long long prof_steps = 0;
    std::string prof_name;
    ddif_prof_class cls_res[6] = {};

    struct Live { size_t bytes; int first, last; size_t off; };
    std::vector<Live> lives;
    std::map<const void*, int> fake2id;
    bool dry = false;
    size_t dry_next = 0;
    int arena_next = 0;
    char* arena = nullptr;
    size_t arena_bytes = 0, unaliased_bytes = 0;
    void use(const void* p);

    struct Tap { std::string name; Tensor t; int op; bool cond_only; };
    std::vector<Tap> taps;
    void tap(const std::string& name, const Tensor& t, bool cond_only = false);
    int forward_taps(const float* x, const float* t_host, const float* sc, float* out, int n, const int* ids, float* const* dst, hipStream_t s);
    ~Plan();
    int build();
    int build_impl();
    template <typename T>
    int dalloc(T** p, size_t n);
    int alloc_tensor(Tensor* t, int C, int H, int W, bool step_act = false);
    int add_conv(std::vector<Op>& prog, const ConvSpec& s, Tensor* out);
    int ensure_tb(int rows);
    int time_rows(const float* t_host, int rows, hipStream_t s);
    void run_prog(std::vector<Op>& prog, hipStream_t s, const StepCtx& ctx, bool prof);
    int n_conv3_f16 = 0;
    int n_conv3_b1 = 0;
    int n_conv3 = 0, n_conv3_x3 = 0;
    bool op_timing_done = false;

    struct TrainMod {
        enum Kind { STEM, FILM, RES, ATTN, DOWN, UP, DEC, FINAL } kind = STEM;
        std::string key;
        Tensor in, out;
        Tensor t[12];
        float* mask = nullptr;
        float* scale = nullptr;
        float* ctx = nullptr;
        float* la_part = nullptr;
        int slot = -1;
        int lev = 0;
        bool has_res = false;
        bool pushes_feat = false;
        int skip_from = -1;
    };
    std::vector<TrainMod> tmods;
    std::vector<Tensor> cenc_pad;
    std::map<std::string, float*> grad_slots;
    std::vector<std::function<void(hipStream_t)>> bwd;
    struct TrainScratch;
    std::shared_ptr<TrainScratch> ts;
    hipStream_t wg_stream = nullptr;
    hipEvent_t wg_fork = nullptr, wg_join = nullptr, side_read = nullptr, a_free[3] = {nullptr, nullptr, nullptr};
    bool wg_async = false;
    bool side_pending = false;
    hipStream_t train_fork(hipStream_t main);
    void train_join(hipStream_t main);
    float* d_loss = nullptr;
    float* dtb = nullptr;
    float* taux = nullptr;
    float* d_net_out = nullptr;
    int build_backward();
    int train_step(const float* x0, const float* noise, const float* a_h, const float* s_h, const float* t_h, const float* sc, float* loss_dev, float* pred,
                   hipStream_t s, const ddif_objective_rows* rows = nullptr, float* recon = nullptr);
    int train_bind(int n, const char* const* keys, float* const* grads);
    int train_forward_backward(const float* x, const float* t_h, const float* sc, const float* target, float* loss_dev, float* pred, hipStream_t s);
    int train_core(const float* t_h, bool has_sc, const float* target_nhwc, float* loss_dev, float* pred, hipStream_t s, const float* p2w = nullptr);
    int train_backward(const float* target_nhwc, float upstream, float* loss_dev, hipStream_t s, const float* p2w = nullptr);
    float* vtarget = nullptr;
    float* obj_rows = nullptr;
    int objective_rows(const ddif_objective_rows* rows, bool need_p2, hipStream_t s);
    int recon(const float* src_nhwc, float* out, bool nchw, hipStream_t s);
    void train_set_stem_source(const float* sc_nhwc);
    int time_rows_aux(const float* t_host, int rows, float* aux, hipStream_t s);

    int train_set_dropout(int site, const float* mask_nchw, hipStream_t s);
    int train_set_droppath(const float* scales_host, hipStream_t s);
    int train_get_dropout(int site, float* mask_nchw, hipStream_t s);
    int train_get_droppath(float* scales_dev, hipStream_t s);
    int train_random_masks(uint64_t seed, uint64_t tile0, float p_drop, float p_path, hipStream_t s);
    int set_cond(const float* cond, hipStream_t s);
    int forward(const float* x, const float* t_host, const float* sc, float* out, hipStream_t s);
    int run_sampler(int kind, int n_steps, const float* const* tabs_host, int n_tabs, const ddif_pred_tables* pred_tabs, const float* t_model, const float* xT,
                    const float* noise, uint64_t seed, uint64_t tile0, float lo, float hi, int do_clamp, float* out, hipStream_t s);
    void drop_graphs();
    int sample_ddpm(const ddif_ddpm_tables* t, const ddif_pred_tables* pt, const float* xT, const float* noise, uint64_t seed, uint64_t tile0,
                    float lo, float hi, int do_clamp, float* out, hipStream_t s);
    int sample_ddim(const ddif_ddim_tables* t, const ddif_pred_tables* pt, const float* xT, const float* noise, uint64_t seed, uint64_t tile0,
                    float lo, float hi, int do_clamp, float* out, hipStream_t s);
    int sample_dpmpp(const ddif_dpm_tables* t, const float* xT, float lo, float hi, int do_clamp, float* out,
                     hipStream_t s);
    int q_sample_forward(const float* x0, const float* noise, const float* a_h, const float* s_h, const float* t_h,
                         const float* sc, float* pred, hipStream_t s, const ddif_objective_rows* rows = nullptr, float* recon_out = nullptr);
};

}
```

### dif-pan_amd/csrc/kernels_lafuse.h

```cpp
#pragma once
#include "ddif_dev.h"

namespace ddif {

struct LaFuseArgs {
    const float* in0;
    const float* in1;
    int c0, c1;
    int B, H, W, b0;
    const double* st0;
    int np0;
    const double* st1;
    int np1;
    const float* gamma;
    const float* beta;
    const float* dw_w;
    const float* wq;
    int nchq;
    const float* bq;
    const float* wmix;
    long long wmix_bstride;
    int nch_mix;
    const float* bias;
    float* out;
    int dout;
    long long* dbg;
    int xcd;
};

template <int TH, int TW, int NBQ, int NBA>
struct LaFuseGeom {
    static constexpr int NPX = TH * TW, NWV = NPX / 32;
    static constexpr int HH = TH + 2, HW = TW + 2;
    static constexpr int LDH = 24;
    static constexpr int LDQ = 20;
    static constexpr int LDX = 28;
    static constexpr int APS = 60;
    static constexpr int HS = HH * HW * LDH, AQ = NPX * LDQ, AX = NPX * LDX;
    static constexpr int NPC = 2 * NBQ + 3 * NBA;
    static constexpr int WC = NPC * 256;
    static constexpr int NPF = 6 * NBA;
    static constexpr int FM = 2 * NPF * 256;
    static constexpr int AP = NPX * APS;
    static constexpr int FEA = 32 * NBQ;
    static constexpr int TAB = 2 * FEA + 9 * FEA + FEA + 32 * NBA;
    static constexpr int CST = 2 * NWV * 32 * 2;
    static constexpr int MAIN = ((HS + AQ + AX + WC) > AP ? (HS + AQ + AX + WC) : AP) + FM;
    static constexpr size_t smem = (size_t)(MAIN + TAB + CST) * sizeof(float);
};

__device__ __forceinline__ void row_pair_swap(float* x, float* y) {
#ifndef DDIF_EMU
    asm volatile("s_nop 1\n\tv_permlane16_swap_b32 %0, %1\n\ts_nop 1" : "+v"(*x), "+v"(*y));
#endif
}
template <bool PAIR = true>
__device__ __forceinline__ float half_allmax(float v) {
#ifdef DDIF_EMU
#pragma unroll
    for (int m = 1; m <= (PAIR ? 16 : 8); m <<= 1) v = fmaxf(v, __shfl_xor(v, m));
    return v;
#else
    v = fmaxf(v, __builtin_bit_cast(float, __builtin_amdgcn_update_dpp(0, __builtin_bit_cast(int, v), 0xB1, 0xf, 0xf, false)));
    v = fmaxf(v, __builtin_bit_cast(float, __builtin_amdgcn_update_dpp(0, __builtin_bit_cast(int, v), 0x4E, 0xf, 0xf, false)));
    v = fmaxf(v, __builtin_bit_cast(float, __builtin_amdgcn_update_dpp(0, __builtin_bit_cast(int, v), 0x124, 0xf, 0xf, false)));
    v = fmaxf(v, __builtin_bit_cast(float, __builtin_amdgcn_update_dpp(0, __builtin_bit_cast(int, v), 0x128, 0xf, 0xf, false)));
    if constexpr (!PAIR) return v;
    float x = v, y = v;
    row_pair_swap(&x, &y);
    return fmaxf(x, y);
#endif
}
template <bool PAIR = true>
__device__ __forceinline__ float half_allsum(float v) {
#ifdef DDIF_EMU
#pragma unroll
    for (int m = 1; m <= (PAIR ? 16 : 8); m <<= 1) v += __shfl_xor(v, m);
    return v;
#else
    v += __builtin_bit_cast(float, __builtin_amdgcn_update_dpp(0, __builtin_bit_cast(int, v), 0xB1, 0xf, 0xf, false));
    v += __builtin_bit_cast(float, __builtin_amdgcn_update_dpp(0, __builtin_bit_cast(int, v), 0x4E, 0xf, 0xf, false));
    v += __builtin_bit_cast(float, __builtin_amdgcn_update_dpp(0, __builtin_bit_cast(int, v), 0x124, 0xf, 0xf, false));
    v += __builtin_bit_cast(float, __builtin_amdgcn_update_dpp(0, __builtin_bit_cast(int, v), 0x128, 0xf, 0xf, false));
    if constexpr (!PAIR) return v;
    float x = v, y = v;
    row_pair_swap(&x, &y);
    return x + y;
#endif
}
#ifdef DDIF_EMU
#define DDIF_WAVE_LDS_SYNC() __syncthreads()
#else
#define DDIF_WAVE_LDS_SYNC() __builtin_amdgcn_fence(__ATOMIC_ACQ_REL, "wavefront")
#endif

template <int TH, int TW, int NBQ, int NBA, int ABL = 0>
__global__ __launch_bounds__(TH * TW * 2) void linattn_fused_kernel(LaFuseArgs a) {
    using G = LaFuseGeom<TH, TW, NBQ, NBA>;
    constexpr int NW = G::NWV, NTHR = 64 * NW;
    static_assert((TH * TW == 256 || TH * TW == 128) && (TH == 16 || TH == 32 || TH == 64), "a workgroup owns 256 or 128 pixels = whole columns of the sample");
    static_assert(TH != 64 || NW % 2 == 0, "64-row columns span a wave pair");
    constexpr int HH = G::HH, HW = G::HW, LDH = G::LDH, LDQ = G::LDQ, LDX = G::LDX, APS = G::APS, FEA = G::FEA;
    constexpr int NCH = 2 * NBQ;
    constexpr int NIT = (HH * HW * 4 + NTHR - 1) / NTHR;
    constexpr int NPC = G::NPC, NPF = G::NPF;
    constexpr int WIT = (NPC + NW - 1) / NW, FIT = (NPF + NW - 1) / NW;
    constexpr float L2E = 1.4426950408889634f;
    constexpr bool PAIRDW = (NBQ == 2 && NBA == 1);

    dd_touch_kernargs<sizeof(LaFuseArgs)>();
    DDIF_DYN_SMEM(smem);
    float* Hs = reinterpret_cast<float*>(smem);
    float* Aq = Hs + G::HS;
    float* Ax = Aq + G::AQ;
    float* Wc = Ax + G::AX;
    float* Ap = Hs;
    float* Fm = Hs + G::MAIN - G::FM;
    float* GB = Hs + G::MAIN;
    float* DW = GB + 2 * FEA;
    float* BQ = DW + 9 * FEA;
    float* BO = BQ + FEA;
    float* Cst = BO + 32 * NBA;

    const int tid = threadIdx.x, lane = tid & 63;
#ifdef DDIF_EMU
    const int wave = tid >> 6;
#else
    const int wave = __builtin_amdgcn_readfirstlane(tid >> 6);
#endif
    const int h = lane >> 5, j = lane & 31;
    [[maybe_unused]] int dbg_n = 0;
    auto stamp = [&]() {
#ifndef DDIF_EMU
        if ((ABL & 64) && a.dbg && tid == 0 && dbg_n < 127) a.dbg[blockIdx.x * 128 + dbg_n++] = (long long)__builtin_amdgcn_s_memtime();
#endif
    };
    const int nstrips = (a.W + TW - 1) / TW;
    const int nwork = a.B * nstrips;
    int w0, w1;
    wg_work_range(nwork, &w0, &w1, a.xcd);
    if (w0 >= w1) return;

    const int c4 = tid & 3;
    float4 raw[NIT];
    unsigned rok = 0;
    auto load_raw = [&](int b, int x0, int k) {
        const int cb = 16 * k;
        const bool s0 = cb < a.c0;
        const float* src = s0 ? a.in0 + cb + 4 * c4 : a.in1 + (cb - a.c0) + 4 * c4;
        const int cs = s0 ? a.c0 : a.c1;
        rok = 0;
#pragma unroll
        for (int it = 0; it < NIT; ++it) {
            const int pix = (tid + it * NTHR) >> 2;
            const bool in = pix < HH * HW;
            const int pc = in ? pix : HH * HW - 1;
            const int y = pc / HW - 1, x = x0 + pc % HW - 1;
            const bool ok = in & (y >= 0) & (y < a.H) & (x >= 0) & (x < a.W);
            rok |= (ok ? 1u : 0u) << it;
            const int yc = y < 0 ? 0 : (y >= a.H ? a.H - 1 : y), xc = x < 0 ? 0 : (x >= a.W ? a.W - 1 : x);
            if (ABL & 1) raw[it] = make_float4(0.5f, -0.25f, 0.125f, 1.f);
            else raw[it] = *reinterpret_cast<const float4*>(src + ((size_t)(b * a.H + yc) * a.W + xc) * cs);
        }
    };
    float4 wst[WIT];
    auto load_weights = [&](const float* wmix_b, int k) {
#pragma unroll
        for (int i = 0; i < WIT; ++i) {
            const int pc = wave + NW * i;
            const int p = pc < NPC ? pc : NPC - 1;
            const float* src;
            if (p < 2 * NBQ) src = a.wq + ((size_t)(((p >> 1) * a.nchq + (k >> 1)) * 2 + (k & 1)) * 2 + (p & 1)) * 256;
            else src = wmix_b + ((size_t)((((p - 2 * NBQ) / 3) * a.nch_mix + ((NCH + k) >> 1)) * 2 + (k & 1)) * 3 + (p - 2 * NBQ) % 3) * 256;
            wst[i] = (ABL & 2) ? make_float4(1e-3f, 2e-3f, 3e-3f, (float)k) : *reinterpret_cast<const float4*>(src + lane * 4);
        }
    };
    auto store_weights = [&]() {
#pragma unroll
        for (int i = 0; i < WIT; ++i)
            if (wave + NW * i < NPC) *reinterpret_cast<float4*>(&Wc[(wave + NW * i) * 256 + lane * 4]) = wst[i];
    };
    float4 fst[FIT];
    auto load_mix = [&](const float* wmix_b, int nb) {
#pragma unroll
        for (int i = 0; i < FIT; ++i) {
            const int pc = wave + NW * i;
            const int p = pc < NPF ? pc : NPF - 1;
            const float* src = wmix_b + ((size_t)(((p / 6) * a.nch_mix + nb) * 2 + (p % 6) / 3) * 3 + p % 3) * 256;
            fst[i] = (ABL & 2) ? make_float4(1e-3f, 2e-3f, 3e-3f, (float)nb) : *reinterpret_cast<const float4*>(src + lane * 4);
        }
    };
    auto store_mix = [&](int par) {
#pragma unroll
        for (int i = 0; i < FIT; ++i)
            if (wave + NW * i < NPF) *reinterpret_cast<float4*>(&Fm[(par * NPF + wave + NW * i) * 256 + lane * 4]) = fst[i];
    };

    int gn_b = -1;
    float mean = 0.f, rstd = 1.f;
    GnPartials gp0;
    {
        const int b = a.b0 + w0 / nstrips;
        gn_load_partials(a.st0, a.np0, a.st1, a.np1, b, &gp0);
        load_raw(b, (w0 % nstrips) * TW, 0);
    }
    {
        constexpr int NDW = (9 * FEA + NTHR - 1) / NTHR, NG = (FEA + NTHR - 1) / NTHR;
        static_assert(32 * NBA <= NTHR, "output bias table: one pass");
        float tg[NG], tb[NG], tq[NG], tdw[NDW];
#pragma unroll
        for (int k = 0; k < NG; ++k) {
            const int i = tid + k * NTHR, ic = i < FEA ? i : FEA - 1;
            tg[k] = a.gamma[ic];
            tb[k] = a.beta[ic];
            tq[k] = a.bq[ic];
        }
        const float to = a.bias[tid < a.dout ? tid : a.dout - 1];
#pragma unroll
        for (int k = 0; k < NDW; ++k) {
            const int i = tid + k * NTHR;
            tdw[k] = a.dw_w[i < 9 * FEA ? i : 9 * FEA - 1];
        }
#pragma unroll
        for (int k = 0; k < NG; ++k) {
            const int i = tid + k * NTHR;
            if (i < FEA) {
                GB[i] = tg[k];
                GB[FEA + i] = tb[k];
                BQ[i] = tq[k];
            }
        }
        if (tid < 32 * NBA) BO[tid] = tid < a.dout ? to : 0.f;
#pragma unroll
        for (int k = 0; k < NDW; ++k) {
            const int i = tid + k * NTHR;
            if (i < 9 * FEA) DW[i] = tdw[k];
        }
    }
    {
        const int b = a.b0 + w0 / nstrips;
        gn_reduce_partials(gp0, a.st0, a.np0, a.st1, a.np1, b, (double)FEA * a.H * a.W, &mean, &rstd);
        gn_b = b;
    }
    __syncthreads();

    for (int work = w0; work < w1; ++work) {
        const int bl = work / nstrips, b = a.b0 + bl, x0 = (work - bl * nstrips) * TW;
        if (b != gn_b) {
            gn_finalize_wave(a.st0, a.np0, a.st1, a.np1, b, (double)FEA * a.H * a.W, &mean, &rstd);
            gn_b = b;
        }
        f32x16 accq[NBQ], acca[NBA];
#pragma unroll
        for (int nb = 0; nb < NBQ; ++nb)
#pragma unroll
            for (int r = 0; r < 16; ++r) accq[nb][r] = 0.f;
#pragma unroll
        for (int nb = 0; nb < NBA; ++nb)
#pragma unroll
            for (int r = 0; r < 16; ++r) acca[nb][r] = 0.f;
        const float* wmix_b = a.wmix + (size_t)b * a.wmix_bstride;
        if constexpr (!(ABL & 16)) load_mix(wmix_b, 0);

#pragma unroll 1
        for (int k = 0; k < NCH; ++k) {
            stamp();
            load_weights(wmix_b, k);
            {
                const float4 gq = *reinterpret_cast<const float4*>(&GB[16 * k + 4 * c4]);
                const float4 bq4 = *reinterpret_cast<const float4*>(&GB[FEA + 16 * k + 4 * c4]);
                float ga[4], gb[4];
#pragma unroll
                for (int i = 0; i < 4; ++i) {
                    ga[i] = (&gq.x)[i] * rstd;
                    gb[i] = (&bq4.x)[i] - mean * ga[i];
                }
#pragma unroll
                for (int it = 0; it < NIT; ++it) {
                    const bool ok = (rok >> it) & 1u;
                    const int pix = (tid + it * NTHR) >> 2;
                    float4 v;
                    v.x = ok ? fmaf(raw[it].x, ga[0], gb[0]) : 0.f;
                    v.y = ok ? fmaf(raw[it].y, ga[1], gb[1]) : 0.f;
                    v.z = ok ? fmaf(raw[it].z, ga[2], gb[2]) : 0.f;
                    v.w = ok ? fmaf(raw[it].w, ga[3], gb[3]) : 0.f;
                    if (pix < HH * HW) *reinterpret_cast<float4*>(&Hs[pix * LDH + 4 * c4]) = v;
                }
            }
            stamp();
            if (k + 1 < NCH) {
                load_raw(b, x0, k + 1);
            } else {
                const int wn = work + 1 < w1 ? work + 1 : work;
                const int bn = wn / nstrips;
                load_raw(a.b0 + bn, (wn - bn * nstrips) * TW, 0);
            }
            __syncthreads();
            stamp();
            if constexpr (PAIRDW) {
              if (!(ABL & 8)) {
                const int p0 = (tid >> 2) * 2, x = p0 / TH, y = p0 % TH;
                float sa[4] = {0.f, 0.f, 0.f, 0.f}, sb[4] = {0.f, 0.f, 0.f, 0.f};
                float4 wprev[3], wcur[3];
#pragma unroll
                for (int r = 0; r < 4; ++r) {
                    float4 hv[3];
#pragma unroll
                    for (int tx = 0; tx < 3; ++tx) {
                        hv[tx] = *reinterpret_cast<const float4*>(&Hs[((y + r) * HW + x + tx) * LDH + 4 * c4]);
                        if (r > 0) wprev[tx] = wcur[tx];
                        if (r < 3) wcur[tx] = *reinterpret_cast<const float4*>(&DW[(3 * r + tx) * FEA + 16 * k + 4 * c4]);
                    }
#pragma unroll
                    for (int tx = 0; tx < 3; ++tx) {
                        if (r < 3) {
                            sa[0] = fmaf(hv[tx].x, wcur[tx].x, sa[0]);
                            sa[1] = fmaf(hv[tx].y, wcur[tx].y, sa[1]);
                            sa[2] = fmaf(hv[tx].z, wcur[tx].z, sa[2]);
                            sa[3] = fmaf(hv[tx].w, wcur[tx].w, sa[3]);
                        }
                        if (r > 0) {
                            sb[0] = fmaf(hv[tx].x, wprev[tx].x, sb[0]);
                            sb[1] = fmaf(hv[tx].y, wprev[tx].y, sb[1]);
                            sb[2] = fmaf(hv[tx].z, wprev[tx].z, sb[2]);
                            sb[3] = fmaf(hv[tx].w, wprev[tx].w, sb[3]);
                        }
                    }
                    if (r == 1 || r == 2) {
                        const int p = p0 + (r - 1);
                        unsigned h01, m01, l01, h23, m23, l23;
                        dd_split3_pair(hv[1].x, hv[1].y, &h01, &m01, &l01);
                        dd_split3_pair(hv[1].z, hv[1].w, &h23, &m23, &l23);
                        *reinterpret_cast<uint2*>(&Ax[p * LDX + 2 * c4]) = make_uint2(h01, h23);
                        *reinterpret_cast<uint2*>(&Ax[p * LDX + 8 + 2 * c4]) = make_uint2(m01, m23);
                        *reinterpret_cast<uint2*>(&Ax[p * LDX + 16 + 2 * c4]) = make_uint2(l01, l23);
                    }
                    DDIF_SCHED_FENCE();
                }
#pragma unroll
                for (int it = 0; it < 2; ++it) {
                    const int p = p0 + it;
                    const float* sv = it ? sb : sa;
                    unsigned h01, l01, h23, l23;
                    dd_split2_pair(sv[0] * DDIF_F16_ASCALE, sv[1] * DDIF_F16_ASCALE, &h01, &l01);
                    dd_split2_pair(sv[2] * DDIF_F16_ASCALE, sv[3] * DDIF_F16_ASCALE, &h23, &l23);
                    *reinterpret_cast<uint2*>(&Aq[p * LDQ + 2 * c4]) = make_uint2(h01, h23);
                    *reinterpret_cast<uint2*>(&Aq[p * LDQ + 8 + 2 * c4]) = make_uint2(l01, l23);
                }
            }
            } else {
#pragma unroll
            for (int it = 0; it < ((ABL & 8) ? 0 : 2); ++it) {
                const int item = tid + it * NTHR, p = item >> 2;
                const int x = p / TH, y = p % TH;
                float s0 = 0.f, s1 = 0.f, s2 = 0.f, s3 = 0.f;
                float4 cen = make_float4(0.f, 0.f, 0.f, 0.f);
#pragma unroll
                for (int ty = 0; ty < 3; ++ty) {
                    float4 hv[3], wk[3];
#pragma unroll
                    for (int tx = 0; tx < 3; ++tx) {
                        hv[tx] = *reinterpret_cast<const float4*>(&Hs[((y + ty) * HW + x + tx) * LDH + 4 * c4]);
                        wk[tx] = *reinterpret_cast<const float4*>(&DW[(3 * ty + tx) * FEA + 16 * k + 4 * c4]);
                    }
#pragma unroll
                    for (int tx = 0; tx < 3; ++tx) {
                        s0 = fmaf(hv[tx].x, wk[tx].x, s0);
                        s1 = fmaf(hv[tx].y, wk[tx].y, s1);
                        s2 = fmaf(hv[tx].z, wk[tx].z, s2);
                        s3 = fmaf(hv[tx].w, wk[tx].w, s3);
                    }
                    if (ty == 1) cen = hv[1];
                    DDIF_SCHED_FENCE();
                }
                unsigned h01, l01, h23, l23;
                dd_split2_pair(s0 * DDIF_F16_ASCALE, s1 * DDIF_F16_ASCALE, &h01, &l01);
                dd_split2_pair(s2 * DDIF_F16_ASCALE, s3 * DDIF_F16_ASCALE, &h23, &l23);
                *reinterpret_cast<uint2*>(&Aq[p * LDQ + 2 * c4]) = make_uint2(h01, h23);
                *reinterpret_cast<uint2*>(&Aq[p * LDQ + 8 + 2 * c4]) = make_uint2(l01, l23);
                unsigned m01, m23;
                dd_split3_pair(cen.x, cen.y, &h01, &m01, &l01);
                dd_split3_pair(cen.z, cen.w, &h23, &m23, &l23);
                *reinterpret_cast<uint2*>(&Ax[p * LDX + 2 * c4]) = make_uint2(h01, h23);
                *reinterpret_cast<uint2*>(&Ax[p * LDX + 8 + 2 * c4]) = make_uint2(m01, m23);
                *reinterpret_cast<uint2*>(&Ax[p * LDX + 16 + 2 * c4]) = make_uint2(l01, l23);
            }
            }
            store_weights();
            stamp();
            __syncthreads();
            stamp();
            {
                const int p = 32 * wave + j;
                float4 xq[2], xr[3];
#pragma unroll
                for (int pl = 0; pl < 2; ++pl) xq[pl] = *reinterpret_cast<const float4*>(&Aq[p * LDQ + pl * 8 + 4 * h]);
#pragma unroll
                for (int pl = 0; pl < 3; ++pl) xr[pl] = *reinterpret_cast<const float4*>(&Ax[p * LDX + pl * 8 + 4 * h]);
#pragma unroll
                for (int nb = 0; nb < NBQ; ++nb) {
                    const float4 f0 = *reinterpret_cast<const float4*>(&Wc[(2 * nb + 0) * 256 + lane * 4]);
                    const float4 f1 = *reinterpret_cast<const float4*>(&Wc[(2 * nb + 1) * 256 + lane * 4]);
                    f32x16 c = accq[nb];
                    if (ABL & 4) {
                        c[0] += f1.x * xq[0].x + f0.y * xq[1].y;
                        accq[nb] = c;
                        continue;
                    }
                    c = DDIF_MFMA_32x32x16_F16(xq[0], f1, c);
                    c = DDIF_MFMA_32x32x16_F16(xq[1], f0, c);
                    c = DDIF_MFMA_32x32x16_F16(xq[0], f0, c);
                    accq[nb] = c;
                }
#pragma unroll
                for (int nb = 0; nb < NBA; ++nb) {
                    float4 f[3];
#pragma unroll
                    for (int pl = 0; pl < 3; ++pl) f[pl] = *reinterpret_cast<const float4*>(&Wc[(2 * NBQ + 3 * nb + pl) * 256 + lane * 4]);
                    f32x16 c = acca[nb];
                    if (ABL & 4) {
                        c[0] += f[2].x * xr[0].x + f[1].y * xr[1].y + f[0].z * xr[2].z;
                        acca[nb] = c;
                        continue;
                    }
                    c = DDIF_MFMA_32x32x16_BF16(f[2], xr[0], c);
                    c = DDIF_MFMA_32x32x16_BF16(f[0], xr[2], c);
                    c = DDIF_MFMA_32x32x16_BF16(f[1], xr[1], c);
                    c = DDIF_MFMA_32x32x16_BF16(f[1], xr[0], c);
                    c = DDIF_MFMA_32x32x16_BF16(f[0], xr[1], c);
                    c = DDIF_MFMA_32x32x16_BF16(f[0], xr[0], c);
                    acca[nb] = c;
                }
            }
            stamp();
        }

        constexpr int NCW = (TH == 16) ? 2 : 1;
        constexpr int RPC = 16 / NCW;
        constexpr int TLD = 36;
        float* Tw = Ap + wave * (32 * TLD);
#pragma unroll
        for (int nb = 0; nb < ((ABL & 16) ? 0 : NBQ); ++nb) {
            DDIF_SCHED_FENCE();
            float e[16], mx[NCW], sm[NCW];
            float* Cs = Cst + (nb & 1) * (NW * 32 * 2);
            const float bj = BQ[32 * nb + j];
#pragma unroll
            for (int r = 0; r < 16; ++r) e[r] = fmaf(accq[nb][r], DDIF_F16_OSCALE, bj);
#pragma unroll
            for (int cg = 0; cg < NCW; ++cg) {
                float m = e[cg * RPC];
#pragma unroll
                for (int r = 1; r < RPC; ++r) m = fmaxf(m, e[cg * RPC + r]);
                m = fmaxf(m, __shfl_xor(m, 32));
                float sacc = 0.f;
#pragma unroll
                for (int r = 0; r < RPC; ++r) {
                    const float ex = dd_exp2_fast((e[cg * RPC + r] - m) * L2E);
                    e[cg * RPC + r] = ex;
                    sacc += ex;
                }
                sacc += __shfl_xor(sacc, 32);
                mx[cg] = m;
                sm[cg] = sacc;
            }
            if constexpr (TH == 64) {
                if (h == 0) *reinterpret_cast<float2*>(&Cs[(wave * 32 + j) * 2]) = make_float2(mx[0], sm[0]);
            }
            store_mix(nb & 1);
            if (nb + 1 < NBQ) load_mix(wmix_b, nb + 1);
            __syncthreads();
            float fac[NCW];
            if constexpr (TH == 64) {
                const float2 o = *reinterpret_cast<const float2*>(&Cs[((wave ^ 1) * 32 + j) * 2]);
                const float M = fmaxf(mx[0], o.x);
                const float cme = dd_exp2_fast((mx[0] - M) * L2E), cpt = dd_exp2_fast((o.x - M) * L2E);
                const float S = (wave & 1) ? (o.y * cpt + sm[0] * cme) : (sm[0] * cme + o.y * cpt);
                fac[0] = cme * dd_rcp_fast(S);
            } else {
#pragma unroll
                for (int cg = 0; cg < NCW; ++cg) fac[cg] = dd_rcp_fast(sm[cg]);
            }
            if (nb > 0) DDIF_WAVE_LDS_SYNC();
#pragma unroll
            for (int r = 0; r < 16; ++r)
                Tw[((r >> 2) * 8 + 4 * h + (r & 3)) * TLD + j] = e[r] * fac[r / RPC];
            DDIF_WAVE_LDS_SYNC();
            const float* Fb = Fm + (nb & 1) * NPF * 256 + lane * 4;
#pragma unroll
            for (int k16 = 0; k16 < 2; ++k16) {
                const float4 t0 = *reinterpret_cast<const float4*>(&Tw[j * TLD + 16 * k16 + 8 * h]);
                const float4 t1 = *reinterpret_cast<const float4*>(&Tw[j * TLD + 16 * k16 + 8 * h + 4]);
                unsigned hh[4], mm[4], ll[4];
                dd_split3_pair(t0.x, t0.y, &hh[0], &mm[0], &ll[0]);
                dd_split3_pair(t0.z, t0.w, &hh[1], &mm[1], &ll[1]);
                dd_split3_pair(t1.x, t1.y, &hh[2], &mm[2], &ll[2]);
                dd_split3_pair(t1.z, t1.w, &hh[3], &mm[3], &ll[3]);
                float4 xp[3];
                xp[0] = make_float4(__builtin_bit_cast(float, hh[0]), __builtin_bit_cast(float, hh[1]), __builtin_bit_cast(float, hh[2]), __builtin_bit_cast(float, hh[3]));
                xp[1] = make_float4(__builtin_bit_cast(float, mm[0]), __builtin_bit_cast(float, mm[1]), __builtin_bit_cast(float, mm[2]), __builtin_bit_cast(float, mm[3]));
                xp[2] = make_float4(__builtin_bit_cast(float, ll[0]), __builtin_bit_cast(float, ll[1]), __builtin_bit_cast(float, ll[2]), __builtin_bit_cast(float, ll[3]));
#pragma unroll
                for (int na = 0; na < NBA; ++na) {
                    float4 f[3];
#pragma unroll
                    for (int pl = 0; pl < 3; ++pl) f[pl] = *reinterpret_cast<const float4*>(&Fb[((na * 2 + k16) * 3 + pl) * 256]);
                    f32x16 c = acca[na];
                    if (ABL & 4) {
                        c[0] += f[2].x * xp[0].x + f[1].y * xp[1].y + f[0].z * xp[2].z;
                        acca[na] = c;
                        continue;
                    }
                    c = DDIF_MFMA_32x32x16_BF16(f[2], xp[0], c);
                    c = DDIF_MFMA_32x32x16_BF16(f[0], xp[2], c);
                    c = DDIF_MFMA_32x32x16_BF16(f[1], xp[1], c);
                    c = DDIF_MFMA_32x32x16_BF16(f[1], xp[0], c);
                    c = DDIF_MFMA_32x32x16_BF16(f[0], xp[1], c);
                    c = DDIF_MFMA_32x32x16_BF16(f[0], xp[0], c);
                    acca[na] = c;
                }
            }
        }
        DDIF_SCHED_FENCE();
        stamp();
        {
            const int p = 32 * wave + j, x = x0 + p / TH, y = p % TH;
            if (x < a.W) {
                float* o = a.out + ((size_t)(b * a.H + y) * a.W + x) * a.dout;
#pragma unroll
                for (int na = 0; na < NBA; ++na)
#pragma unroll
                    for (int g = 0; g < 4; ++g) {
                        const int co = 32 * na + 8 * g + 4 * h;
                        if (co < a.dout) {
                            const float4 bo = *reinterpret_cast<const float4*>(&BO[co]);
                            if (!(ABL & 32) || acca[na][4 * g] == 12345.678f)
                                *reinterpret_cast<float4*>(o + co) =
                                    make_float4(acca[na][4 * g + 0] + bo.x, acca[na][4 * g + 1] + bo.y, acca[na][4 * g + 2] + bo.z, acca[na][4 * g + 3] + bo.w);
                        }
                    }
            }
        }
        __syncthreads();
    }
}

}
```

### dif-pan_amd/csrc/kernels_lafuse8.h

```cpp
#pragma once
#include "kernels_lafuse.h"

namespace ddif {

template <int NBQ>
struct LaFuse8Geom {
    static constexpr int FEA = 32 * NBQ, NCHK = FEA / 64, NS = FEA / 16;
    static constexpr int HW = 6, HH = 10, NHP = HW * HH;
    static constexpr int LDH = 68;
    static constexpr int LDQ = 68;
    static constexpr int LDX = 100;
    static constexpr int LDP = NS * 24 + 4;
    static constexpr int HS = NHP * LDH, AQ = 32 * LDQ, AX = 32 * LDX, AP = 32 * LDP;
    static constexpr int MAIN = (HS + AQ + AX) > AP ? (HS + AQ + AX) : AP;
    static constexpr int RED = 4 * 64 * 16;
    static constexpr int TAB = 2 * FEA + 9 * FEA + FEA + 128;
    static constexpr size_t smem = (size_t)(MAIN + RED + TAB) * sizeof(float);
};

__device__ __forceinline__ float oct_allmax(float v) {
#ifdef DDIF_EMU
#pragma unroll
    for (int m = 1; m <= 4; m <<= 1) v = fmaxf(v, __shfl_xor(v, m));
    return v;
#else
    v = fmaxf(v, __builtin_bit_cast(float, __builtin_amdgcn_update_dpp(0, __builtin_bit_cast(int, v), 0xB1, 0xf, 0xf, false)));
    v = fmaxf(v, __builtin_bit_cast(float, __builtin_amdgcn_update_dpp(0, __builtin_bit_cast(int, v), 0x4E, 0xf, 0xf, false)));
    v = fmaxf(v, __builtin_bit_cast(float, __builtin_amdgcn_update_dpp(0, __builtin_bit_cast(int, v), 0x141, 0xf, 0xf, false)));
    return v;
#endif
}
__device__ __forceinline__ float oct_allsum(float v) {
#ifdef DDIF_EMU
#pragma unroll
    for (int m = 1; m <= 4; m <<= 1) v += __shfl_xor(v, m);
    return v;
#else
    v += __builtin_bit_cast(float, __builtin_amdgcn_update_dpp(0, __builtin_bit_cast(int, v), 0xB1, 0xf, 0xf, false));
    v += __builtin_bit_cast(float, __builtin_amdgcn_update_dpp(0, __builtin_bit_cast(int, v), 0x4E, 0xf, 0xf, false));
    v += __builtin_bit_cast(float, __builtin_amdgcn_update_dpp(0, __builtin_bit_cast(int, v), 0x141, 0xf, 0xf, false));
    return v;
#endif
}

template <int NBQ, int ABL = 0>
__global__ __launch_bounds__(512) void linattn8_fused_kernel(LaFuseArgs a) {
    using G = LaFuse8Geom<NBQ>;
    constexpr int FEA = G::FEA, NCHK = G::NCHK, NS = G::NS, HW = G::HW, HH = G::HH, NHP = G::NHP;
    constexpr int LDH = G::LDH, LDQ = G::LDQ, LDX = G::LDX, LDP = G::LDP;
    constexpr int NSH = NS / 2;
    constexpr int NR0 = NSH / 2, NR1 = NSH - NR0;
    constexpr float L2E = 1.4426950408889634f;
    static_assert(NBQ == 8 || NBQ == 6, "256 or 192 feature channels");

    dd_touch_kernargs<sizeof(LaFuseArgs)>();
    DDIF_DYN_SMEM(smem);
    float* Hs = reinterpret_cast<float*>(smem);
    float* Aq = Hs + G::HS;
    float* Ax = Aq + G::AQ;
    float* Ap = Hs;
    float* Red = Hs + G::MAIN;
    float* GB = Red + G::RED;
    float* DW = GB + 2 * FEA;
    float* BQ = DW + 9 * FEA;
    float* BO = BQ + FEA;

    const int tid = threadIdx.x, lane = tid & 63;
#ifdef DDIF_EMU
    const int wave = tid >> 6;
#else
    const int wave = __builtin_amdgcn_readfirstlane(tid >> 6);
#endif
    const int h = lane >> 5, j = lane & 31;
    [[maybe_unused]] int dbg_n = 0;
    auto stamp = [&]() {
#ifndef DDIF_EMU
        if ((ABL & 64) && a.dbg && tid == 0 && dbg_n < 63) a.dbg[blockIdx.x * 64 + dbg_n++] = (long long)__builtin_amdgcn_s_memtime();
#endif
    };
    stamp();
    const int nwork = a.B * 2;
    int w0, w1;
    wg_work_range(nwork, &w0, &w1, a.xcd);
    if (w0 >= w1) return;

    const int c4 = tid & 15;
    const int nr = wave & 3, kh = wave >> 2;
    const bool qw = wave < NBQ;

    float4 raw[2];
    unsigned rok = 0;
    auto load_raw = [&](int b, int x0, int k) {
        const int cb = 64 * k;
        const bool s0 = cb < a.c0;
        const float* src = s0 ? a.in0 + cb + 4 * c4 : a.in1 + (cb - a.c0) + 4 * c4;
        const int cs = s0 ? a.c0 : a.c1;
        rok = 0;
#pragma unroll
        for (int it = 0; it < 2; ++it) {
            const int pix = (tid + it * 512) >> 4;
            const bool in = pix < NHP;
            const int pc = in ? pix : NHP - 1;
            const int y = pc / HW - 1, x = x0 + pc % HW - 1;
            const bool ok = in & (y >= 0) & (y < 8) & (x >= 0) & (x < 8);
            rok |= (ok ? 1u : 0u) << it;
            const int yc = y < 0 ? 0 : (y > 7 ? 7 : y), xc = x < 0 ? 0 : (x > 7 ? 7 : x);
            raw[it] = *reinterpret_cast<const float4*>(src + ((size_t)(b * 8 + yc) * 8 + xc) * cs);
        }
    };

    int gn_b = -1;
    float mean = 0.f, rstd = 1.f;
    GnPartials gp0;
    {
        const int b = a.b0 + (w0 >> 1);
        gn_load_partials(a.st0, a.np0, a.st1, a.np1, b, &gp0);
        load_raw(b, (w0 & 1) * 4, 0);
    }
    {
        constexpr int NDW = (9 * FEA + 511) / 512;
        const int ic = tid < FEA ? tid : FEA - 1, io = tid < 128 ? tid : 127;
        const float tg = a.gamma[ic], tb = a.beta[ic], tq = a.bq[ic], to = a.bias[io];
        float tdw[NDW];
#pragma unroll
        for (int k = 0; k < NDW; ++k) {
            const int i = tid + k * 512;
            tdw[k] = a.dw_w[i < 9 * FEA ? i : 9 * FEA - 1];
        }
        if (tid < FEA) {
            GB[tid] = tg;
            GB[FEA + tid] = tb;
            BQ[tid] = tq;
        }
        if (tid < 128) BO[tid] = to;
#pragma unroll
        for (int k = 0; k < NDW; ++k) {
            const int i = tid + k * 512;
            if (i < 9 * FEA) DW[i] = tdw[k];
        }
    }
    {
        const int b = a.b0 + (w0 >> 1);
        gn_reduce_partials(gp0, a.st0, a.np0, a.st1, a.np1, b, (double)FEA * 64, &mean, &rstd);
        gn_b = b;
    }
    __syncthreads();
    stamp();

    for (int work = w0; work < w1; ++work) {
        const int b = a.b0 + (work >> 1), x0 = (work & 1) * 4;
        if (b != gn_b) {
            gn_finalize_wave(a.st0, a.np0, a.st1, a.np1, b, (double)FEA * 64, &mean, &rstd);
            gn_b = b;
        }
        f32x16 accq, acca;
#pragma unroll
        for (int r = 0; r < 16; ++r) {
            accq[r] = 0.f;
            acca[r] = 0.f;
        }
        const float* wmix_b = a.wmix + (size_t)b * a.wmix_bstride;
        const float* wq_w = a.wq + (size_t)(qw ? wave : 0) * a.nchq * (2 * 2 * 256);
        const float* wr_w = wmix_b + ((size_t)nr * a.nch_mix + NBQ + kh) * (2 * 3 * 256);
        unsigned lo4 = (unsigned)lane * 4u;
#ifndef DDIF_EMU
        asm volatile("" : "+v"(lo4));
#endif

#pragma unroll 1
        for (int k = 0; k < NCHK; ++k) {
            float4 wqr[4][2], wrr[2][3];
            const float* wqk = wq_w + (size_t)k * (2 * 2 * 2 * 256);
            const float* wrk = wr_w + (size_t)k * (2 * 2 * 3 * 256);
#pragma unroll
            for (int sl = 0; sl < 4; ++sl)
#pragma unroll
                for (int pl = 0; pl < 2; ++pl) wqr[sl][pl] = *reinterpret_cast<const float4*>(wqk + ((sl >> 1) * 4 + (sl & 1) * 2 + pl) * 256 + lo4);
#pragma unroll
            for (int t = 0; t < 2; ++t)
#pragma unroll
                for (int pl = 0; pl < 3; ++pl) wrr[t][pl] = *reinterpret_cast<const float4*>(wrk + (t * 3 + pl) * 256 + lo4);
            if (ABL & 128) stamp();
            {
                const float4 gq = *reinterpret_cast<const float4*>(&GB[64 * k + 4 * c4]);
                const float4 bq4 = *reinterpret_cast<const float4*>(&GB[FEA + 64 * k + 4 * c4]);
                float ga[4], gb[4];
#pragma unroll
                for (int i = 0; i < 4; ++i) {
                    ga[i] = (&gq.x)[i] * rstd;
                    gb[i] = (&bq4.x)[i] - mean * ga[i];
                }
#pragma unroll
                for (int it = 0; it < 2; ++it) {
                    const bool ok = (rok >> it) & 1u;
                    const int pix = (tid + it * 512) >> 4;
                    float4 v;
                    v.x = ok ? fmaf(raw[it].x, ga[0], gb[0]) : 0.f;
                    v.y = ok ? fmaf(raw[it].y, ga[1], gb[1]) : 0.f;
                    v.z = ok ? fmaf(raw[it].z, ga[2], gb[2]) : 0.f;
                    v.w = ok ? fmaf(raw[it].w, ga[3], gb[3]) : 0.f;
                    if (pix < NHP) *reinterpret_cast<float4*>(&Hs[pix * LDH + 4 * c4]) = v;
                }
            }
            if (ABL & 128) stamp();
            if (k + 1 < NCHK) {
                load_raw(b, x0, k + 1);
            } else {
                const int wn = work + 1 < w1 ? work + 1 : work;
                load_raw(a.b0 + (wn >> 1), (wn & 1) * 4, 0);
            }
            __syncthreads();
            if (ABL & 128) stamp();
            {
                const int p = tid >> 4, xl = p >> 3, y = p & 7;
                float s0 = 0.f, s1 = 0.f, s2 = 0.f, s3 = 0.f;
                float4 cen = make_float4(0.f, 0.f, 0.f, 0.f);
#pragma unroll
                for (int ty = 0; ty < 3; ++ty) {
                    float4 hv[3], wk[3];
#pragma unroll
                    for (int tx = 0; tx < 3; ++tx) {
                        hv[tx] = *reinterpret_cast<const float4*>(&Hs[((y + ty) * HW + xl + tx) * LDH + 4 * c4]);
                        wk[tx] = *reinterpret_cast<const float4*>(&DW[(3 * ty + tx) * FEA + 64 * k + 4 * c4]);
                    }
#pragma unroll
                    for (int tx = 0; tx < 3; ++tx) {
                        s0 = fmaf(hv[tx].x, wk[tx].x, s0);
                        s1 = fmaf(hv[tx].y, wk[tx].y, s1);
                        s2 = fmaf(hv[tx].z, wk[tx].z, s2);
                        s3 = fmaf(hv[tx].w, wk[tx].w, s3);
                    }
                    if (ty == 1) cen = hv[1];
                }
                const int sl = c4 >> 2, e2 = (c4 & 3) * 2;
                unsigned h01, l01, h23, l23, m01, m23;
                dd_split2_pair(s0 * DDIF_F16_ASCALE, s1 * DDIF_F16_ASCALE, &h01, &l01);
                dd_split2_pair(s2 * DDIF_F16_ASCALE, s3 * DDIF_F16_ASCALE, &h23, &l23);
                *reinterpret_cast<uint2*>(&Aq[p * LDQ + sl * 16 + e2]) = make_uint2(h01, h23);
                *reinterpret_cast<uint2*>(&Aq[p * LDQ + sl * 16 + 8 + e2]) = make_uint2(l01, l23);
                dd_split3_pair(cen.x, cen.y, &h01, &m01, &l01);
                dd_split3_pair(cen.z, cen.w, &h23, &m23, &l23);
                *reinterpret_cast<uint2*>(&Ax[p * LDX + sl * 24 + e2]) = make_uint2(h01, h23);
                *reinterpret_cast<uint2*>(&Ax[p * LDX + sl * 24 + 8 + e2]) = make_uint2(m01, m23);
                *reinterpret_cast<uint2*>(&Ax[p * LDX + sl * 24 + 16 + e2]) = make_uint2(l01, l23);
            }
            if (ABL & 128) stamp();
            __syncthreads();
            if (ABL & 128) stamp();
            if (qw) {
#pragma unroll
                for (int sl = 0; sl < 4; ++sl) {
                    const float4 x0q = *reinterpret_cast<const float4*>(&Aq[j * LDQ + sl * 16 + 4 * h]);
                    const float4 x1q = *reinterpret_cast<const float4*>(&Aq[j * LDQ + sl * 16 + 8 + 4 * h]);
                    accq = DDIF_MFMA_32x32x16_F16(wqr[sl][1], x0q, accq);
                    accq = DDIF_MFMA_32x32x16_F16(wqr[sl][0], x1q, accq);
                    accq = DDIF_MFMA_32x32x16_F16(wqr[sl][0], x0q, accq);
                }
            }
#pragma unroll
            for (int t = 0; t < 2; ++t) {
                const int sl = 2 * kh + t;
                float4 xr[3];
#pragma unroll
                for (int pl = 0; pl < 3; ++pl) xr[pl] = *reinterpret_cast<const float4*>(&Ax[j * LDX + sl * 24 + pl * 8 + 4 * h]);
                acca = DDIF_MFMA_32x32x16_BF16(wrr[t][2], xr[0], acca);
                acca = DDIF_MFMA_32x32x16_BF16(wrr[t][0], xr[2], acca);
                acca = DDIF_MFMA_32x32x16_BF16(wrr[t][1], xr[1], acca);
                acca = DDIF_MFMA_32x32x16_BF16(wrr[t][1], xr[0], acca);
                acca = DDIF_MFMA_32x32x16_BF16(wrr[t][0], xr[1], acca);
                acca = DDIF_MFMA_32x32x16_BF16(wrr[t][0], xr[0], acca);
            }
            if (ABL & 128) stamp();
        }
        stamp();

        float4 wm0[NR0][3], wm1[NR1][3];
        auto mix_piece = [&](int sl, int pl) {
            return *reinterpret_cast<const float4*>(wmix_b + ((size_t)((((nr * a.nch_mix + (sl >> 1)) * 2 + (sl & 1)) * 3 + pl)) * 256) + lo4);
        };
#pragma unroll
        for (int i = 0; i < NR0; ++i)
#pragma unroll
            for (int pl = 0; pl < 3; ++pl) wm0[i][pl] = mix_piece(kh * NSH + i, pl);
#pragma unroll
        for (int i = 0; i < NR1; ++i)
#pragma unroll
            for (int pl = 0; pl < 3; ++pl) wm1[i][pl] = mix_piece(kh * NSH + NR0 + i, pl);

        float e[16];
        if (qw) {
#pragma unroll
            for (int g = 0; g < 4; ++g) {
                const float4 bq4 = *reinterpret_cast<const float4*>(&BQ[32 * wave + 8 * g + 4 * h]);
#pragma unroll
                for (int i = 0; i < 4; ++i) {
                    const float q = fmaf(accq[4 * g + i], DDIF_F16_OSCALE, (&bq4.x)[i]);
                    const float m = oct_allmax(q);
                    const float ex = dd_exp2_fast((q - m) * L2E);
                    e[4 * g + i] = ex * dd_rcp_fast(oct_allsum(ex));
                }
            }
        }
        __syncthreads();
        if (qw) {
#pragma unroll
            for (int g = 0; g < 4; ++g) {
                unsigned h01, m01, l01, h23, m23, l23;
                dd_split3_pair(e[4 * g + 0], e[4 * g + 1], &h01, &m01, &l01);
                dd_split3_pair(e[4 * g + 2], e[4 * g + 3], &h23, &m23, &l23);
                float* d = &Ap[j * LDP + (2 * wave + (g >> 1)) * 24 + (g & 1) * 4 + 2 * h];
                *reinterpret_cast<uint2*>(d) = make_uint2(h01, h23);
                *reinterpret_cast<uint2*>(d + 8) = make_uint2(m01, m23);
                *reinterpret_cast<uint2*>(d + 16) = make_uint2(l01, l23);
            }
        }
        __syncthreads();
        stamp();
        auto mix_step = [&](int sl, const float4* f) {
            float4 xp[3];
#pragma unroll
            for (int pl = 0; pl < 3; ++pl) xp[pl] = *reinterpret_cast<const float4*>(&Ap[j * LDP + sl * 24 + pl * 8 + 4 * h]);
            acca = DDIF_MFMA_32x32x16_BF16(f[2], xp[0], acca);
            acca = DDIF_MFMA_32x32x16_BF16(f[0], xp[2], acca);
            acca = DDIF_MFMA_32x32x16_BF16(f[1], xp[1], acca);
            acca = DDIF_MFMA_32x32x16_BF16(f[1], xp[0], acca);
            acca = DDIF_MFMA_32x32x16_BF16(f[0], xp[1], acca);
            acca = DDIF_MFMA_32x32x16_BF16(f[0], xp[0], acca);
        };
#pragma unroll
        for (int i = 0; i < NR0; ++i) mix_step(kh * NSH + i, wm0[i]);
#pragma unroll
        for (int i = 0; i < NR1; ++i) mix_step(kh * NSH + NR0 + i, wm1[i]);
        stamp();
        if (kh == 1) {
#pragma unroll
            for (int g = 0; g < 4; ++g)
                *reinterpret_cast<float4*>(&Red[((nr * 64 + lane) * 4 + g) * 4]) = make_float4(acca[4 * g + 0], acca[4 * g + 1], acca[4 * g + 2], acca[4 * g + 3]);
        }
        __syncthreads();
        if (kh == 0) {
            const int xl = j >> 3, y = j & 7;
            float* o = a.out + ((size_t)(b * 8 + y) * 8 + x0 + xl) * a.dout + 32 * nr + 4 * h;
#pragma unroll
            for (int g = 0; g < 4; ++g) {
                const float4 o1 = *reinterpret_cast<const float4*>(&Red[((nr * 64 + lane) * 4 + g) * 4]);
                const float4 bo = *reinterpret_cast<const float4*>(&BO[32 * nr + 8 * g + 4 * h]);
                *reinterpret_cast<float4*>(o + 8 * g) = make_float4((acca[4 * g + 0] + o1.x) + bo.x, (acca[4 * g + 1] + o1.y) + bo.y, (acca[4 * g + 2] + o1.z) + bo.z,
                                                                   (acca[4 * g + 3] + o1.w) + bo.w);
            }
        }
        stamp();
    }
}

}
```

Baseline: 0.07867 MP/s.

## Use f16x2 residual projection in linear-attention fusion and add channel-split variant

Packs the attn_res weights into an f16 hi/lo form and, when the GroupNorm absmax bound shows activations fit in f16 range, runs the residual projection with 3 f16 MFMAs per slice instead of 6 bf16x3 MFMAs. The split activation tile in LDS shrinks from three planes to two. It also adds a channel-split variant for 16-row images that doubles the waves per workgroup when the grid would underfill the CUs, so each wave pair owns half the output channels. The cost is template instantiation growth and reduced precision headroom, which is guarded by the range check.

```diff
diff --git a/dif-pan_amd/csrc/ddif_la.cpp b/dif-pan_amd/csrc/ddif_la.cpp
--- a/dif-pan_amd/csrc/ddif_la.cpp
+++ b/dif-pan_amd/csrc/ddif_la.cpp
@@ -5,15 +5,34 @@
 namespace ddif {
 
 namespace {
-template <int TH, int TW, int NBQ, int NBA>
-int la_launch1(const LaFuseArgs& a, int grid, hipStream_t s, bool prepare_only) {
-    using G = LaFuseGeom<TH, TW, NBQ, NBA>;
-    auto fn = linattn_fused_kernel<TH, TW, NBQ, NBA>;
+template <int TH, int TW, int NBQ, int NBA, bool RF16, int CS = 1>
+int la_launch2(const LaFuseArgs& a, int grid, hipStream_t s, bool prepare_only) {
+    using G = LaFuseGeom<TH, TW, NBQ, NBA, RF16, CS>;
+    auto fn = linattn_fused_kernel<TH, TW, NBQ, NBA, 0, RF16, CS>;
     if (prepare_only) {
         DDIF_HIPCHK(hipFuncSetAttribute(reinterpret_cast<const void*>(fn), hipFuncAttributeMaxDynamicSharedMemorySize, (int)G::smem));
         return 0;
     }
-    hipLaunchKernelGGL(fn, dim3(grid), dim3(2 * TH * TW), G::smem, s, a);
+    hipLaunchKernelGGL(fn, dim3(grid), dim3(64 * G::NWV), G::smem, s, a);
+    return 0;
+}
+template <int TH, int TW, int NBQ, int NBA>
+int la_launch1(const LaFuseArgs& a, int grid, hipStream_t s, bool prepare_only) {
+    return a.wres16 ? la_launch2<TH, TW, NBQ, NBA, true>(a, grid, s, prepare_only) : la_launch2<TH, TW, NBQ, NBA, false>(a, grid, s, prepare_only);
+}
+template <int NBQ>
+int la_launch_cs(const LaFuseArgs& a, int grid, hipStream_t s, bool prepare_only) {
+    return a.wres16 ? la_launch2<16, 4, NBQ, 2, true, 2>(a, grid, s, prepare_only) : la_launch2<16, 4, NBQ, 2, false, 2>(a, grid, s, prepare_only);
+}
+template <int NBQ, bool RF16>
+int la8_launch1(const LaFuseArgs& a, int grid, hipStream_t s, bool prepare_only) {
+    using G = LaFuse8Geom<NBQ, RF16>;
+    auto fn = linattn8_fused_kernel<NBQ, 0, RF16>;
+    if (prepare_only) {
+        DDIF_HIPCHK(hipFuncSetAttribute(reinterpret_cast<const void*>(fn), hipFuncAttributeMaxDynamicSharedMemorySize, (int)G::smem));
+        return 0;
+    }
+    hipLaunchKernelGGL(fn, dim3(grid), dim3(512), G::smem, s, a);
     return 0;
 }
 template <int TH, int TW>
@@ -38,9 +57,15 @@
     if (H == 16 && fea == 192 && dout == 64 && la6) return true;
     return (H == 64 || H == 32 || H == 16) && fea % 32 == 0 && fea >= 64 && fea <= 128 && dout % 32 == 0 && dout >= 32 && dout <= 64;
 }
-int lafuse_strip(int H, int nw) { return 32 * nw / H; }
-int lafuse_launch(const LaFuseArgs& a, int grid, hipStream_t s, bool prepare_only, int nw) {
+int lafuse_strip(int H, int nw, int cs) { return 32 * nw / cs / H; }
+bool lafuse_csplit_supported(int H, int fea, int dout) { return H == 16 && (fea == 128 || fea == 192) && dout == 64 && lafuse_supported(H, fea, dout); }
+int lafuse_launch(const LaFuseArgs& a, int grid, hipStream_t s, bool prepare_only, int nw, int cs) {
     const int nbq = (a.c0 + a.c1) / 32, nba = a.dout / 32;
+    if (cs == 2) {
+        if (nw == 4 && a.H == 16 && nba == 2 && nbq == 4) return la_launch_cs<4>(a, grid, s, prepare_only);
+        if (nw == 4 && a.H == 16 && nba == 2 && nbq == 6) return la_launch_cs<6>(a, grid, s, prepare_only);
+        return fail(DDIF_ERR_INVALID, "linattn_fused: no channel-split instantiation for H = %d, %d q blocks / %d output blocks", a.H, nbq, nba);
+    }
     if (nw == 4) {
         if (a.H == 64) return la_launch_t<64, 2>(a, nbq, nba, grid, s, prepare_only);
         if (a.H == 32) return la_launch_t<32, 4>(a, nbq, nba, grid, s, prepare_only);
@@ -58,24 +83,8 @@
 }
 int lafuse8_launch(const LaFuseArgs& a, int grid, hipStream_t s, bool prepare_only) {
     const int nbq = (a.c0 + a.c1) / 32;
-    if (nbq == 8) {
-        auto fn = linattn8_fused_kernel<8>;
-        if (prepare_only) {
-            DDIF_HIPCHK(hipFuncSetAttribute(reinterpret_cast<const void*>(fn), hipFuncAttributeMaxDynamicSharedMemorySize, (int)LaFuse8Geom<8>::smem));
-            return 0;
-        }
-        hipLaunchKernelGGL(fn, dim3(grid), dim3(512), LaFuse8Geom<8>::smem, s, a);
-        return 0;
-    }
-    if (nbq == 6) {
-        auto fn = linattn8_fused_kernel<6>;
-        if (prepare_only) {
-            DDIF_HIPCHK(hipFuncSetAttribute(reinterpret_cast<const void*>(fn), hipFuncAttributeMaxDynamicSharedMemorySize, (int)LaFuse8Geom<6>::smem));
-            return 0;
-        }
-        hipLaunchKernelGGL(fn, dim3(grid), dim3(512), LaFuse8Geom<6>::smem, s, a);
-        return 0;
-    }
+    if (nbq == 8) return a.wres16 ? la8_launch1<8, true>(a, grid, s, prepare_only) : la8_launch1<8, false>(a, grid, s, prepare_only);
+    if (nbq == 6) return a.wres16 ? la8_launch1<6, true>(a, grid, s, prepare_only) : la8_launch1<6, false>(a, grid, s, prepare_only);
     return fail(DDIF_ERR_INVALID, "linattn8_fused: %d feature channels", a.c0 + a.c1);
 }
 
diff --git a/dif-pan_amd/csrc/ddif_net.cpp b/dif-pan_amd/csrc/ddif_net.cpp
--- a/dif-pan_amd/csrc/ddif_net.cpp
+++ b/dif-pan_amd/csrc/ddif_net.cpp
@@ -422,6 +422,10 @@
         if (wr) {
             vec_off[ci + ".attn_res.weight"] = b.add(wr->v.data(), wr->v.size());
             rec_copy(RF_COPY, ci + ".attn_res.weight", "", vec_off[ci + ".attn_res.weight"], wr->v.size());
+            if (wr->shape.size() == 4 && wr->shape[1] % 32 == 0) {
+                const size_t off = pack_conv_f16(b, wr->v.data(), (int)wr->shape[0], (int)wr->shape[1], 1, 32);
+                if (off != (size_t)-1) vec_off[ci + ".attn_res.weight.f16"] = off;
+            }
         }
         if (wo && bo) {
             const int co = (int)wo->shape[0], fea = (int)wo->shape[1];
diff --git a/dif-pan_amd/csrc/ddif_plan.cpp b/dif-pan_amd/csrc/ddif_plan.cpp
--- a/dif-pan_amd/csrc/ddif_plan.cpp
+++ b/dif-pan_amd/csrc/ddif_plan.cpp
@@ -1243,31 +1243,48 @@
         a.bias = pm->bias;
         a.out = amix->p;
         a.dout = pm->cout;
+        {
+            static const bool rf16 = env_flag("DDIF_LA_RES_F16", true);
+            const float* w16 = V(ci + ".attn_res.weight.f16");
+            auto ig = net.vec_absmax.find(D.pn_g), ib = net.vec_absmax.find(D.pn_b);
+            const bool okr = ig != net.vec_absmax.end() && ib != net.vec_absmax.end() &&
+                             std::sqrt((double)fea * Hl * Wl) * ig->second + ib->second < DDIF_F16_AMAX;
+            a.wres16 = (rf16 && w16 && okr) ? w16 : nullptr;
+            a.nchr = fea / 32;
+        }
         int la_nw = 8;
         if (!la8) {
             static const int nw_env = env_int("DDIF_LA_NW", 0);
             const long wg8 = (long)B * ((Wl + lafuse_strip(Hl, 8) - 1) / lafuse_strip(Hl, 8));
             la_nw = nw_env == 4 || nw_env == 8 ? nw_env : (wg8 < num_cus() ? 4 : 8);
         }
-        if (!p.dry) DDIF_TRY(la8 ? lafuse8_launch(a, 1, nullptr, true) : lafuse_launch(a, 1, nullptr, true, la_nw));
-        const int nstrips = la8 ? 2 : (Wl + lafuse_strip(Hl, la_nw) - 1) / lafuse_strip(Hl, la_nw);
+        int la_cs = 1;
+        if (!la8 && la_nw == 4) {
+            static const bool cs_env = env_flag("DDIF_LA_CSPLIT", true);
+            const long wg4 = (long)B * ((Wl + lafuse_strip(Hl, 4) - 1) / lafuse_strip(Hl, 4));
+            if (cs_env && lafuse_csplit_supported(Hl, fea, pm->cout) && 2 * wg4 <= num_cus()) la_cs = 2;
+        }
+        if (!p.dry) DDIF_TRY(la8 ? lafuse8_launch(a, 1, nullptr, true) : lafuse_launch(a, 1, nullptr, true, la_nw, la_cs));
+        const int nstrips = la8 ? 2 : (Wl + lafuse_strip(Hl, la_nw, la_cs) - 1) / lafuse_strip(Hl, la_nw, la_cs);
         long cap = num_cus();
         if (g_debug_grid_cap > 0 && g_debug_grid_cap < cap) cap = g_debug_grid_cap;
         Op op;
         op.name = la8 ? "linattn8_fused" : "linattn_fused";
         {
             char lb[160];
-            snprintf(lb, sizeof lb, "linattn_fused GN+dw3x3+q.1+softmax_H+attn_out+res %d+%d->%d @%dx%d", cur.C, skip.C, pm->cout, Hl, Wl);
+            snprintf(lb, sizeof lb, "linattn_fused GN+dw3x3+q.1+softmax_H+attn_out+res(%s) %d+%d->%d @%dx%d", a.wres16 ? "f16x2" : "bf16x3", cur.C, skip.C, pm->cout, Hl, Wl);
             op.label = lb;
         }
+        if (getenv("DDIF_DUMP_PLAN"))
+            fprintf(stderr, "[ddif la] %-34s res=%s nw=%d csplit=%d\n", ci.c_str(), a.wres16 ? "f16x2" : "bf16x3", la_nw, la_cs);
         op.flop = 2.0 * B * Hl * Wl * ((double)fea * fea + 9.0 * fea + 2.0 * fea * pm->cout);
         op.bytes = 4.0 * B * Hl * Wl * ((double)fea + pm->cout);
         op.cls = cls_small(Hl * Wl, 1);
-        op.mfma_w = (3.0 * fea * fea + 6.0 * 2.0 * fea * pm->cout) / ((double)fea * fea + 9.0 * fea + 2.0 * fea * pm->cout);
-        op.run = [a, nstrips, cap, la8, la_nw](hipStream_t st, const StepCtx&) {
+        op.mfma_w = (3.0 * fea * fea + (6.0 + (a.wres16 ? 3.0 : 6.0)) * fea * pm->cout) / ((double)fea * fea + 9.0 * fea + 2.0 * fea * pm->cout);
+        op.run = [a, nstrips, cap, la8, la_nw, la_cs](hipStream_t st, const StepCtx&) {
             const long nw = (long)a.B * nstrips;
             if (la8) (void)lafuse8_launch(a, (int)(nw < cap ? nw : cap), st, false);
-            else (void)lafuse_launch(a, (int)(nw < cap ? nw : cap), st, false, la_nw);
+            else (void)lafuse_launch(a, (int)(nw < cap ? nw : cap), st, false, la_nw, la_cs);
         };
         step.push_back(std::move(op));
         *fused = true;
diff --git a/dif-pan_amd/csrc/ddif_plan.h b/dif-pan_amd/csrc/ddif_plan.h
--- a/dif-pan_amd/csrc/ddif_plan.h
+++ b/dif-pan_amd/csrc/ddif_plan.h
@@ -68,8 +68,9 @@
 extern int g_f16_raw;
 struct LaFuseArgs;
 bool lafuse_supported(int H, int fea, int dout);
-int lafuse_strip(int H, int nw = 8);
-int lafuse_launch(const LaFuseArgs& a, int grid, hipStream_t s, bool prepare_only, int nw = 8);
+int lafuse_strip(int H, int nw = 8, int cs = 1);
+bool lafuse_csplit_supported(int H, int fea, int dout);
+int lafuse_launch(const LaFuseArgs& a, int grid, hipStream_t s, bool prepare_only, int nw = 8, int cs = 1);
 bool lafuse8_supported(int H, int W, int c0, int c1, int dout);
 int lafuse8_launch(const LaFuseArgs& a, int grid, hipStream_t s, bool prepare_only);
 namespace tk {
diff --git a/dif-pan_amd/csrc/kernels_lafuse.h b/dif-pan_amd/csrc/kernels_lafuse.h
--- a/dif-pan_amd/csrc/kernels_lafuse.h
+++ b/dif-pan_amd/csrc/kernels_lafuse.h
@@ -18,6 +18,8 @@
     const float* wq;
     int nchq;
     const float* bq;
+    const float* wres16;
+    int nchr;
     const float* wmix;
     long long wmix_bstride;
     int nch_mix;
@@ -28,20 +30,22 @@
     int xcd;
 };
 
-template <int TH, int TW, int NBQ, int NBA>
+template <int TH, int TW, int NBQ, int NBA, bool RF16 = false, int CS = 1>
 struct LaFuseGeom {
-    static constexpr int NPX = TH * TW, NWV = NPX / 32;
+    static constexpr int NPX = TH * TW, NWV = CS * NPX / 32;
     static constexpr int HH = TH + 2, HW = TW + 2;
     static constexpr int LDH = 24;
     static constexpr int LDQ = 20;
-    static constexpr int LDX = 28;
+    static constexpr int NPR = RF16 ? 2 : 3;
+    static constexpr int LDX = 8 * NPR + 4;
     static constexpr int APS = 60;
     static constexpr int HS = HH * HW * LDH, AQ = NPX * LDQ, AX = NPX * LDX;
-    static constexpr int NPC = 2 * NBQ + 3 * NBA;
+    static constexpr int NPC = 2 * NBQ + NPR * NBA;
     static constexpr int WC = NPC * 256;
     static constexpr int NPF = 6 * NBA;
-    static constexpr int FM = 2 * NPF * 256;
-    static constexpr int AP = NPX * APS;
+    static constexpr int FM = CS == 2 ? 0 : 2 * NPF * 256;
+    static constexpr int TWS = NWV * 32 * 36;
+    static constexpr int AP = CS == 2 ? TWS + NBQ * NPX * APS : NPX * APS;
     static constexpr int FEA = 32 * NBQ;
     static constexpr int TAB = 2 * FEA + 9 * FEA + FEA + 32 * NBA;
     static constexpr int CST = 2 * NWV * 32 * 2;
@@ -94,11 +98,14 @@
 #define DDIF_WAVE_LDS_SYNC() __builtin_amdgcn_fence(__ATOMIC_ACQ_REL, "wavefront")
 #endif
 
-template <int TH, int TW, int NBQ, int NBA, int ABL = 0>
-__global__ __launch_bounds__(TH * TW * 2) void linattn_fused_kernel(LaFuseArgs a) {
-    using G = LaFuseGeom<TH, TW, NBQ, NBA>;
+template <int TH, int TW, int NBQ, int NBA, int ABL = 0, bool RF16 = false, int CS = 1>
+__global__ __launch_bounds__(TH * TW * 2 * CS) void linattn_fused_kernel(LaFuseArgs a) {
+    using G = LaFuseGeom<TH, TW, NBQ, NBA, RF16, CS>;
+    static_assert(CS == 1 || (CS == 2 && TH == 16 && TW == 4 && NBQ % 2 == 0 && NBA % 2 == 0 && ABL == 0), "channel split: 64 pixels of a 16-row image on four waves");
+    constexpr int NBQW = NBQ / CS, NBAW = NBA / CS;
+    constexpr int NPR = G::NPR;
     constexpr int NW = G::NWV, NTHR = 64 * NW;
-    static_assert((TH * TW == 256 || TH * TW == 128) && (TH == 16 || TH == 32 || TH == 64), "a workgroup owns 256 or 128 pixels = whole columns of the sample");
+    static_assert((TH * TW == 256 || TH * TW == 128 || CS == 2) && (TH == 16 || TH == 32 || TH == 64), "a workgroup owns 256 or 128 pixels = whole columns of the sample");
     static_assert(TH != 64 || NW % 2 == 0, "64-row columns span a wave pair");
     constexpr int HH = G::HH, HW = G::HW, LDH = G::LDH, LDQ = G::LDQ, LDX = G::LDX, APS = G::APS, FEA = G::FEA;
     constexpr int NCH = 2 * NBQ;
@@ -129,6 +136,8 @@
     const int wave = __builtin_amdgcn_readfirstlane(tid >> 6);
 #endif
     const int h = lane >> 5, j = lane & 31;
+    const int pb = CS == 2 ? (wave & 1) : wave;
+    const int ch = CS == 2 ? (wave >> 1) : 0;
     [[maybe_unused]] int dbg_n = 0;
     auto stamp = [&]() {
 #ifndef DDIF_EMU
@@ -171,6 +180,7 @@
             const int p = pc < NPC ? pc : NPC - 1;
             const float* src;
             if (p < 2 * NBQ) src = a.wq + ((size_t)(((p >> 1) * a.nchq + (k >> 1)) * 2 + (k & 1)) * 2 + (p & 1)) * 256;
+            else if constexpr (RF16) src = a.wres16 + ((size_t)((((p - 2 * NBQ) >> 1) * a.nchr + (k >> 1)) * 2 + (k & 1)) * 2 + ((p - 2 * NBQ) & 1)) * 256;
             else src = wmix_b + ((size_t)((((p - 2 * NBQ) / 3) * a.nch_mix + ((NCH + k) >> 1)) * 2 + (k & 1)) * 3 + (p - 2 * NBQ) % 3) * 256;
             wst[i] = (ABL & 2) ? make_float4(1e-3f, 2e-3f, 3e-3f, (float)k) : *reinterpret_cast<const float4*>(src + lane * 4);
         }
@@ -250,18 +260,34 @@
             gn_finalize_wave(a.st0, a.np0, a.st1, a.np1, b, (double)FEA * a.H * a.W, &mean, &rstd);
             gn_b = b;
         }
-        f32x16 accq[NBQ], acca[NBA];
-#pragma unroll
-        for (int nb = 0; nb < NBQ; ++nb)
+        f32x16 accq[NBQW], acca[NBAW];
+#pragma unroll
+        for (int nb = 0; nb < NBQW; ++nb)
 #pragma unroll
             for (int r = 0; r < 16; ++r) accq[nb][r] = 0.f;
 #pragma unroll
-        for (int nb = 0; nb < NBA; ++nb)
+        for (int nb = 0; nb < NBAW; ++nb)
 #pragma unroll
             for (int r = 0; r < 16; ++r) acca[nb][r] = 0.f;
         const float* wmix_b = a.wmix + (size_t)b * a.wmix_bstride;
-        if constexpr (!(ABL & 16)) load_mix(wmix_b, 0);
-
+        if constexpr (!(ABL & 16) && CS == 1) load_mix(wmix_b, 0);
+
+        auto store_xn = [&](int p, const float4& v) {
+            if constexpr (RF16) {
+                unsigned h01, l01, h23, l23;
+                dd_split2_pair(v.x * DDIF_F16_ASCALE, v.y * DDIF_F16_ASCALE, &h01, &l01);
+                dd_split2_pair(v.z * DDIF_F16_ASCALE, v.w * DDIF_F16_ASCALE, &h23, &l23);
+                *reinterpret_cast<uint2*>(&Ax[p * LDX + 2 * c4]) = make_uint2(h01, h23);
+                *reinterpret_cast<uint2*>(&Ax[p * LDX + 8 + 2 * c4]) = make_uint2(l01, l23);
+            } else {
+                unsigned h01, m01, l01, h23, m23, l23;
+                dd_split3_pair(v.x, v.y, &h01, &m01, &l01);
+                dd_split3_pair(v.z, v.w, &h23, &m23, &l23);
+                *reinterpret_cast<uint2*>(&Ax[p * LDX + 2 * c4]) = make_uint2(h01, h23);
+                *reinterpret_cast<uint2*>(&Ax[p * LDX + 8 + 2 * c4]) = make_uint2(m01, m23);
+                *reinterpret_cast<uint2*>(&Ax[p * LDX + 16 + 2 * c4]) = make_uint2(l01, l23);
+            }
+        };
 #pragma unroll 1
         for (int k = 0; k < NCH; ++k) {
             stamp();
@@ -327,13 +353,7 @@
                         }
                     }
                     if (r == 1 || r == 2) {
-                        const int p = p0 + (r - 1);
-                        unsigned h01, m01, l01, h23, m23, l23;
-                        dd_split3_pair(hv[1].x, hv[1].y, &h01, &m01, &l01);
-                        dd_split3_pair(hv[1].z, hv[1].w, &h23, &m23, &l23);
-                        *reinterpret_cast<uint2*>(&Ax[p * LDX + 2 * c4]) = make_uint2(h01, h23);
-                        *reinterpret_cast<uint2*>(&Ax[p * LDX + 8 + 2 * c4]) = make_uint2(m01, m23);
-                        *reinterpret_cast<uint2*>(&Ax[p * LDX + 16 + 2 * c4]) = make_uint2(l01, l23);
+                        store_xn(p0 + (r - 1), hv[1]);
                     }
                     DDIF_SCHED_FENCE();
                 }
@@ -350,7 +370,7 @@
             }
             } else {
 #pragma unroll
-            for (int it = 0; it < ((ABL & 8) ? 0 : 2); ++it) {
+            for (int it = 0; it < ((ABL & 8) ? 0 : 4 * TH * TW / NTHR); ++it) {
                 const int item = tid + it * NTHR, p = item >> 2;
                 const int x = p / TH, y = p % TH;
                 float s0 = 0.f, s1 = 0.f, s2 = 0.f, s3 = 0.f;
@@ -378,12 +398,7 @@
                 dd_split2_pair(s2 * DDIF_F16_ASCALE, s3 * DDIF_F16_ASCALE, &h23, &l23);
                 *reinterpret_cast<uint2*>(&Aq[p * LDQ + 2 * c4]) = make_uint2(h01, h23);
                 *reinterpret_cast<uint2*>(&Aq[p * LDQ + 8 + 2 * c4]) = make_uint2(l01, l23);
-                unsigned m01, m23;
-                dd_split3_pair(cen.x, cen.y, &h01, &m01, &l01);
-                dd_split3_pair(cen.z, cen.w, &h23, &m23, &l23);
-                *reinterpret_cast<uint2*>(&Ax[p * LDX + 2 * c4]) = make_uint2(h01, h23);
-                *reinterpret_cast<uint2*>(&Ax[p * LDX + 8 + 2 * c4]) = make_uint2(m01, m23);
-                *reinterpret_cast<uint2*>(&Ax[p * LDX + 16 + 2 * c4]) = make_uint2(l01, l23);
+                store_xn(p, cen);
             }
             }
             store_weights();
@@ -391,54 +406,153 @@
             __syncthreads();
             stamp();
             {
-                const int p = 32 * wave + j;
-                float4 xq[2], xr[3];
+                const int p = 32 * pb + j;
+                float4 xq[2], xr[NPR];
 #pragma unroll
                 for (int pl = 0; pl < 2; ++pl) xq[pl] = *reinterpret_cast<const float4*>(&Aq[p * LDQ + pl * 8 + 4 * h]);
 #pragma unroll
-                for (int pl = 0; pl < 3; ++pl) xr[pl] = *reinterpret_cast<const float4*>(&Ax[p * LDX + pl * 8 + 4 * h]);
-#pragma unroll
-                for (int nb = 0; nb < NBQ; ++nb) {
+                for (int pl = 0; pl < NPR; ++pl) xr[pl] = *reinterpret_cast<const float4*>(&Ax[p * LDX + pl * 8 + 4 * h]);
+#pragma unroll
+                for (int i = 0; i < NBQW; ++i) {
+                    const int nb = ch * NBQW + i;
                     const float4 f0 = *reinterpret_cast<const float4*>(&Wc[(2 * nb + 0) * 256 + lane * 4]);
                     const float4 f1 = *reinterpret_cast<const float4*>(&Wc[(2 * nb + 1) * 256 + lane * 4]);
-                    f32x16 c = accq[nb];
+                    f32x16 c = accq[i];
                     if (ABL & 4) {
                         c[0] += f1.x * xq[0].x + f0.y * xq[1].y;
-                        accq[nb] = c;
+                        accq[i] = c;
                         continue;
                     }
                     c = DDIF_MFMA_32x32x16_F16(xq[0], f1, c);
                     c = DDIF_MFMA_32x32x16_F16(xq[1], f0, c);
                     c = DDIF_MFMA_32x32x16_F16(xq[0], f0, c);
-                    accq[nb] = c;
-                }
-#pragma unroll
-                for (int nb = 0; nb < NBA; ++nb) {
-                    float4 f[3];
-#pragma unroll
-                    for (int pl = 0; pl < 3; ++pl) f[pl] = *reinterpret_cast<const float4*>(&Wc[(2 * NBQ + 3 * nb + pl) * 256 + lane * 4]);
-                    f32x16 c = acca[nb];
+                    accq[i] = c;
+                }
+#pragma unroll
+                for (int i = 0; i < NBAW; ++i) {
+                    const int nb = ch * NBAW + i;
+                    float4 f[NPR];
+#pragma unroll
+                    for (int pl = 0; pl < NPR; ++pl) f[pl] = *reinterpret_cast<const float4*>(&Wc[(2 * NBQ + NPR * nb + pl) * 256 + lane * 4]);
+                    f32x16 c = acca[i];
                     if (ABL & 4) {
-                        c[0] += f[2].x * xr[0].x + f[1].y * xr[1].y + f[0].z * xr[2].z;
-                        acca[nb] = c;
+                        c[0] += f[NPR - 1].x * xr[0].x + f[1].y * xr[1].y + f[0].z * xr[NPR - 1].z;
+                        acca[i] = c;
                         continue;
                     }
-                    c = DDIF_MFMA_32x32x16_BF16(f[2], xr[0], c);
-                    c = DDIF_MFMA_32x32x16_BF16(f[0], xr[2], c);
-                    c = DDIF_MFMA_32x32x16_BF16(f[1], xr[1], c);
-                    c = DDIF_MFMA_32x32x16_BF16(f[1], xr[0], c);
-                    c = DDIF_MFMA_32x32x16_BF16(f[0], xr[1], c);
-                    c = DDIF_MFMA_32x32x16_BF16(f[0], xr[0], c);
-                    acca[nb] = c;
+                    if constexpr (RF16) {
+                        c = DDIF_MFMA_32x32x16_F16(f[1], xr[0], c);
+                        c = DDIF_MFMA_32x32x16_F16(f[0], xr[1], c);
+                        c = DDIF_MFMA_32x32x16_F16(f[0], xr[0], c);
+                    } else {
+                        c = DDIF_MFMA_32x32x16_BF16(f[2], xr[0], c);
+                        c = DDIF_MFMA_32x32x16_BF16(f[0], xr[2], c);
+                        c = DDIF_MFMA_32x32x16_BF16(f[1], xr[1], c);
+                        c = DDIF_MFMA_32x32x16_BF16(f[1], xr[0], c);
+                        c = DDIF_MFMA_32x32x16_BF16(f[0], xr[1], c);
+                        c = DDIF_MFMA_32x32x16_BF16(f[0], xr[0], c);
+                    }
+                    acca[i] = c;
                 }
             }
             stamp();
         }
 
+        if constexpr (RF16) {
+#pragma unroll
+            for (int nb = 0; nb < NBAW; ++nb)
+#pragma unroll
+                for (int r = 0; r < 16; ++r) acca[nb][r] *= DDIF_F16_OSCALE;
+        }
         constexpr int NCW = (TH == 16) ? 2 : 1;
         constexpr int RPC = 16 / NCW;
         constexpr int TLD = 36;
         float* Tw = Ap + wave * (32 * TLD);
+        if constexpr (CS == 2) {
+            static_assert(G::TWS == G::NWV * 32 * TLD, "transpose tiles");
+            float* Pp = Ap + G::TWS;
+            float4 fm[2][NBAW][2][3];
+            auto load_frag = [&](int nb, float4 (*f)[2][3]) {
+#pragma unroll
+                for (int na = 0; na < NBAW; ++na)
+#pragma unroll
+                    for (int k16 = 0; k16 < 2; ++k16)
+#pragma unroll
+                        for (int pl = 0; pl < 3; ++pl)
+                            f[na][k16][pl] = *reinterpret_cast<const float4*>(wmix_b + ((size_t)((((ch * NBAW + na) * a.nch_mix + nb) * 2 + k16) * 3 + pl)) * 256 + lane * 4);
+            };
+            load_frag(0, fm[0]);
+            __syncthreads();
+#pragma unroll
+            for (int i = 0; i < NBQW; ++i) {
+                DDIF_SCHED_FENCE();
+                const int nb = ch * NBQW + i;
+                float e[16], sm[NCW];
+                const float bj = BQ[32 * nb + j];
+#pragma unroll
+                for (int r = 0; r < 16; ++r) e[r] = fmaf(accq[i][r], DDIF_F16_OSCALE, bj);
+#pragma unroll
+                for (int cg = 0; cg < NCW; ++cg) {
+                    float m = e[cg * RPC];
+#pragma unroll
+                    for (int r = 1; r < RPC; ++r) m = fmaxf(m, e[cg * RPC + r]);
+                    m = fmaxf(m, __shfl_xor(m, 32));
+                    float sacc = 0.f;
+#pragma unroll
+                    for (int r = 0; r < RPC; ++r) {
+                        const float ex = dd_exp2_fast((e[cg * RPC + r] - m) * L2E);
+                        e[cg * RPC + r] = ex;
+                        sacc += ex;
+                    }
+                    sacc += __shfl_xor(sacc, 32);
+                    sm[cg] = sacc;
+                }
+                float fac[NCW];
+#pragma unroll
+                for (int cg = 0; cg < NCW; ++cg) fac[cg] = dd_rcp_fast(sm[cg]);
+                if (i > 0) DDIF_WAVE_LDS_SYNC();
+#pragma unroll
+                for (int r = 0; r < 16; ++r) Tw[((r >> 2) * 8 + 4 * h + (r & 3)) * TLD + j] = e[r] * fac[r / RPC];
+                DDIF_WAVE_LDS_SYNC();
+#pragma unroll
+                for (int k16 = 0; k16 < 2; ++k16) {
+                    const float4 t0 = *reinterpret_cast<const float4*>(&Tw[j * TLD + 16 * k16 + 8 * h]);
+                    const float4 t1 = *reinterpret_cast<const float4*>(&Tw[j * TLD + 16 * k16 + 8 * h + 4]);
+                    unsigned hh[4], mm[4], ll[4];
+                    dd_split3_pair(t0.x, t0.y, &hh[0], &mm[0], &ll[0]);
+                    dd_split3_pair(t0.z, t0.w, &hh[1], &mm[1], &ll[1]);
+                    dd_split3_pair(t1.x, t1.y, &hh[2], &mm[2], &ll[2]);
+                    dd_split3_pair(t1.z, t1.w, &hh[3], &mm[3], &ll[3]);
+                    unsigned* d = reinterpret_cast<unsigned*>(&Pp[((pb * NBQ + nb) * 32 + j) * APS + k16 * 24 + 4 * h]);
+                    *reinterpret_cast<uint4*>(d) = make_uint4(hh[0], hh[1], hh[2], hh[3]);
+                    *reinterpret_cast<uint4*>(d + 8) = make_uint4(mm[0], mm[1], mm[2], mm[3]);
+                    *reinterpret_cast<uint4*>(d + 16) = make_uint4(ll[0], ll[1], ll[2], ll[3]);
+                }
+            }
+            __syncthreads();
+#pragma unroll
+            for (int nb = 0; nb < NBQ; ++nb) {
+                if (nb + 1 < NBQ) load_frag(nb + 1, fm[(nb + 1) & 1]);
+#pragma unroll
+                for (int k16 = 0; k16 < 2; ++k16) {
+                    float4 xp[3];
+#pragma unroll
+                    for (int pl = 0; pl < 3; ++pl) xp[pl] = *reinterpret_cast<const float4*>(&Pp[((pb * NBQ + nb) * 32 + j) * APS + k16 * 24 + pl * 8 + 4 * h]);
+#pragma unroll
+                    for (int na = 0; na < NBAW; ++na) {
+                        const float4* f = fm[nb & 1][na][k16];
+                        f32x16 c = acca[na];
+                        c = DDIF_MFMA_32x32x16_BF16(f[2], xp[0], c);
+                        c = DDIF_MFMA_32x32x16_BF16(f[0], xp[2], c);
+                        c = DDIF_MFMA_32x32x16_BF16(f[1], xp[1], c);
+                        c = DDIF_MFMA_32x32x16_BF16(f[1], xp[0], c);
+                        c = DDIF_MFMA_32x32x16_BF16(f[0], xp[1], c);
+                        c = DDIF_MFMA_32x32x16_BF16(f[0], xp[0], c);
+                        acca[na] = c;
+                    }
+                }
+            }
+        } else {
 #pragma unroll
         for (int nb = 0; nb < ((ABL & 16) ? 0 : NBQ); ++nb) {
             DDIF_SCHED_FENCE();
@@ -521,17 +635,18 @@
                 }
             }
         }
+        }
         DDIF_SCHED_FENCE();
         stamp();
         {
-            const int p = 32 * wave + j, x = x0 + p / TH, y = p % TH;
+            const int p = 32 * pb + j, x = x0 + p / TH, y = p % TH;
             if (x < a.W) {
                 float* o = a.out + ((size_t)(b * a.H + y) * a.W + x) * a.dout;
 #pragma unroll
-                for (int na = 0; na < NBA; ++na)
+                for (int na = 0; na < NBAW; ++na)
 #pragma unroll
                     for (int g = 0; g < 4; ++g) {
-                        const int co = 32 * na + 8 * g + 4 * h;
+                        const int co = 32 * (ch * NBAW + na) + 8 * g + 4 * h;
                         if (co < a.dout) {
                             const float4 bo = *reinterpret_cast<const float4*>(&BO[co]);
                             if (!(ABL & 32) || acca[na][4 * g] == 12345.678f)
diff --git a/dif-pan_amd/csrc/kernels_lafuse8.h b/dif-pan_amd/csrc/kernels_lafuse8.h
--- a/dif-pan_amd/csrc/kernels_lafuse8.h
+++ b/dif-pan_amd/csrc/kernels_lafuse8.h
@@ -3,13 +3,14 @@
 
 namespace ddif {
 
-template <int NBQ>
+template <int NBQ, bool RF16 = false>
 struct LaFuse8Geom {
     static constexpr int FEA = 32 * NBQ, NCHK = FEA / 64, NS = FEA / 16;
     static constexpr int HW = 6, HH = 10, NHP = HW * HH;
     static constexpr int LDH = 68;
     static constexpr int LDQ = 68;
-    static constexpr int LDX = 100;
+    static constexpr int NPR = RF16 ? 2 : 3;
+    static constexpr int LDX = 4 * 8 * NPR + 4;
     static constexpr int LDP = NS * 24 + 4;
     static constexpr int HS = NHP * LDH, AQ = 32 * LDQ, AX = 32 * LDX, AP = 32 * LDP;
     static constexpr int MAIN = (HS + AQ + AX) > AP ? (HS + AQ + AX) : AP;
@@ -43,9 +44,10 @@
 #endif
 }
 
-template <int NBQ, int ABL = 0>
+template <int NBQ, int ABL = 0, bool RF16 = false>
 __global__ __launch_bounds__(512) void linattn8_fused_kernel(LaFuseArgs a) {
-    using G = LaFuse8Geom<NBQ>;
+    using G = LaFuse8Geom<NBQ, RF16>;
+    constexpr int NPR = G::NPR;
     constexpr int FEA = G::FEA, NCHK = G::NCHK, NS = G::NS, HW = G::HW, HH = G::HH, NHP = G::NHP;
     constexpr int LDH = G::LDH, LDQ = G::LDQ, LDX = G::LDX, LDP = G::LDP;
     constexpr int NSH = NS / 2;
@@ -161,7 +163,7 @@
         }
         const float* wmix_b = a.wmix + (size_t)b * a.wmix_bstride;
         const float* wq_w = a.wq + (size_t)(qw ? wave : 0) * a.nchq * (2 * 2 * 256);
-        const float* wr_w = wmix_b + ((size_t)nr * a.nch_mix + NBQ + kh) * (2 * 3 * 256);
+        const float* wr_w = RF16 ? a.wres16 + ((size_t)nr * a.nchr + kh) * (2 * 2 * 256) : wmix_b + ((size_t)nr * a.nch_mix + NBQ + kh) * (2 * 3 * 256);
         unsigned lo4 = (unsigned)lane * 4u;
 #ifndef DDIF_EMU
         asm volatile("" : "+v"(lo4));
@@ -169,9 +171,9 @@
 
 #pragma unroll 1
         for (int k = 0; k < NCHK; ++k) {
-            float4 wqr[4][2], wrr[2][3];
+            float4 wqr[4][2], wrr[2][NPR];
             const float* wqk = wq_w + (size_t)k * (2 * 2 * 2 * 256);
-            const float* wrk = wr_w + (size_t)k * (2 * 2 * 3 * 256);
+            const float* wrk = wr_w + (size_t)k * (2 * 2 * NPR * 256);
 #pragma unroll
             for (int sl = 0; sl < 4; ++sl)
 #pragma unroll
@@ -179,7 +181,7 @@
 #pragma unroll
             for (int t = 0; t < 2; ++t)
 #pragma unroll
-                for (int pl = 0; pl < 3; ++pl) wrr[t][pl] = *reinterpret_cast<const float4*>(wrk + (t * 3 + pl) * 256 + lo4);
+                for (int pl = 0; pl < NPR; ++pl) wrr[t][pl] = *reinterpret_cast<const float4*>(wrk + (t * NPR + pl) * 256 + lo4);
             if (ABL & 128) stamp();
             {
                 const float4 gq = *reinterpret_cast<const float4*>(&GB[64 * k + 4 * c4]);
@@ -233,16 +235,23 @@
                     if (ty == 1) cen = hv[1];
                 }
                 const int sl = c4 >> 2, e2 = (c4 & 3) * 2;
-                unsigned h01, l01, h23, l23, m01, m23;
+                [[maybe_unused]] unsigned h01, l01, h23, l23, m01, m23;
                 dd_split2_pair(s0 * DDIF_F16_ASCALE, s1 * DDIF_F16_ASCALE, &h01, &l01);
                 dd_split2_pair(s2 * DDIF_F16_ASCALE, s3 * DDIF_F16_ASCALE, &h23, &l23);
                 *reinterpret_cast<uint2*>(&Aq[p * LDQ + sl * 16 + e2]) = make_uint2(h01, h23);
                 *reinterpret_cast<uint2*>(&Aq[p * LDQ + sl * 16 + 8 + e2]) = make_uint2(l01, l23);
-                dd_split3_pair(cen.x, cen.y, &h01, &m01, &l01);
-                dd_split3_pair(cen.z, cen.w, &h23, &m23, &l23);
-                *reinterpret_cast<uint2*>(&Ax[p * LDX + sl * 24 + e2]) = make_uint2(h01, h23);
-                *reinterpret_cast<uint2*>(&Ax[p * LDX + sl * 24 + 8 + e2]) = make_uint2(m01, m23);
-                *reinterpret_cast<uint2*>(&Ax[p * LDX + sl * 24 + 16 + e2]) = make_uint2(l01, l23);
+                if constexpr (RF16) {
+                    dd_split2_pair(cen.x * DDIF_F16_ASCALE, cen.y * DDIF_F16_ASCALE, &h01, &l01);
+                    dd_split2_pair(cen.z * DDIF_F16_ASCALE, cen.w * DDIF_F16_ASCALE, &h23, &l23);
+                    *reinterpret_cast<uint2*>(&Ax[p * LDX + sl * 16 + e2]) = make_uint2(h01, h23);
+                    *reinterpret_cast<uint2*>(&Ax[p * LDX + sl * 16 + 8 + e2]) = make_uint2(l01, l23);
+                } else {
+                    dd_split3_pair(cen.x, cen.y, &h01, &m01, &l01);
+                    dd_split3_pair(cen.z, cen.w, &h23, &m23, &l23);
+                    *reinterpret_cast<uint2*>(&Ax[p * LDX + sl * 24 + e2]) = make_uint2(h01, h23);
+                    *reinterpret_cast<uint2*>(&Ax[p * LDX + sl * 24 + 8 + e2]) = make_uint2(m01, m23);
+                    *reinterpret_cast<uint2*>(&Ax[p * LDX + sl * 24 + 16 + e2]) = make_uint2(l01, l23);
+                }
             }
             if (ABL & 128) stamp();
             __syncthreads();
@@ -260,19 +269,29 @@
 #pragma unroll
             for (int t = 0; t < 2; ++t) {
                 const int sl = 2 * kh + t;
-                float4 xr[3];
-#pragma unroll
-                for (int pl = 0; pl < 3; ++pl) xr[pl] = *reinterpret_cast<const float4*>(&Ax[j * LDX + sl * 24 + pl * 8 + 4 * h]);
-                acca = DDIF_MFMA_32x32x16_BF16(wrr[t][2], xr[0], acca);
-                acca = DDIF_MFMA_32x32x16_BF16(wrr[t][0], xr[2], acca);
-                acca = DDIF_MFMA_32x32x16_BF16(wrr[t][1], xr[1], acca);
-                acca = DDIF_MFMA_32x32x16_BF16(wrr[t][1], xr[0], acca);
-                acca = DDIF_MFMA_32x32x16_BF16(wrr[t][0], xr[1], acca);
-                acca = DDIF_MFMA_32x32x16_BF16(wrr[t][0], xr[0], acca);
+                float4 xr[NPR];
+#pragma unroll
+                for (int pl = 0; pl < NPR; ++pl) xr[pl] = *reinterpret_cast<const float4*>(&Ax[j * LDX + sl * 8 * NPR + pl * 8 + 4 * h]);
+                if constexpr (RF16) {
+                    acca = DDIF_MFMA_32x32x16_F16(wrr[t][1], xr[0], acca);
+                    acca = DDIF_MFMA_32x32x16_F16(wrr[t][0], xr[1], acca);
+                    acca = DDIF_MFMA_32x32x16_F16(wrr[t][0], xr[0], acca);
+                } else {
+                    acca = DDIF_MFMA_32x32x16_BF16(wrr[t][2], xr[0], acca);
+                    acca = DDIF_MFMA_32x32x16_BF16(wrr[t][0], xr[2], acca);
+                    acca = DDIF_MFMA_32x32x16_BF16(wrr[t][1], xr[1], acca);
+                    acca = DDIF_MFMA_32x32x16_BF16(wrr[t][1], xr[0], acca);
+                    acca = DDIF_MFMA_32x32x16_BF16(wrr[t][0], xr[1], acca);
+                    acca = DDIF_MFMA_32x32x16_BF16(wrr[t][0], xr[0], acca);
+                }
             }
             if (ABL & 128) stamp();
         }
         stamp();
+        if constexpr (RF16) {
+#pragma unroll
+            for (int r = 0; r < 16; ++r) acca[r] *= DDIF_F16_OSCALE;
+        }
 
         float4 wm0[NR0][3], wm1[NR1][3];
         auto mix_piece = [&](int sl, int pl) {
```

Result: faster. 0.08020 MP/s, median of 6 (+1.9%).
